# RMichelsen/VulkanHybridRenderer

Hardware: AMD Instinct MI355X
Metric: Mrays/s (unique rays) + ms/frame, Sponza 1080p RT shadows+AO+SVGF (higher is better)
Workload: dtype f32

## Files before the change

include/vhr_amd.h:

```cpp
#ifndef VHR_AMD_H
#define VHR_AMD_H

#include "vhr_types.h"

#ifdef __cplusplus
extern "C" {
#endif

typedef struct vhr_context vhr_context;
typedef struct vhr_raytracing_execution_context vhr_raytracing_execution_context;
typedef struct vhr_compute_execution_context vhr_compute_execution_context;

enum {
    VHR_OK = 0,
    VHR_ERROR_INVALID_ARGUMENT = -1,
    VHR_ERROR_DEVICE = -2,
    VHR_ERROR_NOT_FOUND = -3,
    VHR_ERROR_OUT_OF_SLOTS = -4,
    VHR_ERROR_GRAPH = -5,
    VHR_ERROR_NO_DEVICE = -6,
    VHR_ERROR_UNSUPPORTED = -7
};

enum {
// ... 185 lines not shown
    uint32_t grid_rows, grid_cols;
    uint32_t col_begin, col_end, row_begin, row_end;
    uint32_t overlap;
    uint32_t halo_rows, halo_cols;
    uint32_t col_cut[VHR_TILE_MAX_GRID + 1], row_cut[VHR_TILE_MAX_GRID][VHR_TILE_MAX_GRID + 1];
} vhr_tile_plan;
typedef struct vhr_rect { uint32_t x0, x1, y0, y1; } vhr_rect;
typedef struct vhr_rect_exchange { int32_t peer; vhr_rect send, recv; } vhr_rect_exchange;
#define VHR_COMM_UNIQUE_ID_BYTES 128
typedef struct vhr_comm vhr_comm;

uint32_t vhr_atrous_overlap(uint32_t atrous_steps);
uint32_t vhr_atrous_output_extent(uint32_t overlap, uint32_t step);
int vhr_strip_plan_make(uint32_t height, uint32_t world, uint32_t rank, uint32_t max_motion_rows, uint32_t atrous_steps, vhr_strip_plan *out);
int vhr_strip_plan_exchanges(const vhr_strip_plan *plan, uint32_t n_rows, vhr_row_exchange out[2]);

int vhr_tile_grid_choose(uint32_t width, uint32_t height, uint32_t world, uint32_t overlap, uint32_t *grid_rows, uint32_t *grid_cols);
int vhr_tile_plan_make(uint32_t width, uint32_t height, uint32_t world, uint32_t rank, uint32_t grid_rows, uint32_t grid_cols, uint32_t max_motion_rows,
                       uint32_t max_motion_cols, uint32_t atrous_steps, vhr_tile_plan *out);
int vhr_tile_plan_make_weighted(uint32_t width, uint32_t height, uint32_t world, uint32_t rank, uint32_t grid_rows, uint32_t grid_cols, uint32_t max_motion_rows,
                                uint32_t max_motion_cols, uint32_t atrous_steps, const uint32_t *cost, uint32_t cost_cols, uint32_t cost_rows, uint32_t cell,
                                vhr_tile_plan *out);
int vhr_tile_plan_exchanges(const vhr_tile_plan *plan, uint32_t halo_rows, uint32_t halo_cols, vhr_rect_exchange *out, uint32_t capacity);
int vhr_tile_plan_replan(const vhr_tile_plan *old_plan, const vhr_tile_plan *new_plan, vhr_rect_exchange *out, uint32_t capacity);

int vhr_comm_use_library(const char *path);
const char *vhr_comm_library(void);
int vhr_comm_get_unique_id(uint8_t out[VHR_COMM_UNIQUE_ID_BYTES]);
int vhr_comm_create(vhr_context *ctx, const vhr_strip_plan *plan, const uint8_t unique_id[VHR_COMM_UNIQUE_ID_BYTES], vhr_comm **out);
int vhr_comm_create_tiled(vhr_context *ctx, const vhr_tile_plan *plan, const uint8_t unique_id[VHR_COMM_UNIQUE_ID_BYTES], vhr_comm **out);
void vhr_comm_destroy(vhr_comm *comm);
const char *vhr_comm_last_error(const vhr_comm *comm);
int vhr_comm_exchange_raytraced(vhr_comm *comm, const char *raytraced_image);
int vhr_comm_start_frame_exchanges(vhr_comm *comm, int32_t history_storage_image, int32_t moments_storage_image, const char *denoised_image,
                                   int32_t root, void *gathered_frame);
int vhr_comm_finish_frame_exchanges(vhr_comm *comm);
int vhr_comm_replan(vhr_comm *comm, const vhr_tile_plan *new_plan, int32_t history_storage_image, int32_t moments_storage_image, int32_t prev_normals_storage_image);

int vhr_set_ray_statistics(vhr_context *ctx, int32_t enable);
int vhr_get_ray_statistics(vhr_context *ctx, uint64_t out[4]);

int vhr_set_option(vhr_context *ctx, const char *key, int32_t value);
int vhr_get_option(vhr_context *ctx, const char *key, int32_t *value);
int32_t vhr_option_count(void);
int vhr_option_info(int32_t index, const char **name, int32_t *default_value, int32_t *min_value, int32_t *max_value);

int vhr_set_kernel_timing(vhr_context *ctx, int32_t kind_mask);
int vhr_get_kernel_time(vhr_context *ctx, int32_t kind, double *total_ms, uint64_t *launches, int32_t reset);

const char *vhr_source_fingerprint(void);
int vhr_debug_wave_lifetimes(vhr_context *ctx, uint32_t *out, uint32_t capacity, uint32_t *count);
int vhr_debug_ray_triangle(vhr_context *ctx, const float *pairs, uint32_t count, uint32_t *hit, float *tuv);
int vhr_debug_triangle_records(vhr_context *ctx, int32_t previous, float *out, uint32_t capacity_triangles, uint32_t *count);
int vhr_get_tile_cost_map(vhr_context *ctx, uint32_t *out, uint32_t cols, uint32_t rows);

int vhr_get_traversal_statistics(vhr_context *ctx, uint64_t out[4]);
int vhr_get_reflection_statistics(vhr_context *ctx, uint64_t out[10]);
int vhr_get_binary64_statistics(vhr_context *ctx, uint64_t out[4]);

int vhr_get_traversal_cycles(vhr_context *ctx, uint64_t out[8]);

int vhr_get_drain_statistics(vhr_context *ctx, uint64_t out[4]);

int vhr_calibration_stream_read(vhr_context *ctx, int32_t storage_image, uint32_t bytes_per_lane);

int vhr_get_build_times(vhr_context *ctx, double out[2]);
int vhr_get_bvh_builder(vhr_context *ctx, int32_t *used);
int vhr_get_bvh_presplit_level(vhr_context *ctx, int32_t *level);
int vhr_get_bvh_frame(vhr_context *ctx, float out[9]);

int vhr_get_bvh_statistics(vhr_context *ctx, uint64_t out[5]);
int vhr_get_bvh_form_checks(vhr_context *ctx, uint64_t out[4]);
int vhr_get_bvh_fingerprint(vhr_context *ctx, uint64_t *out);
int vhr_get_bvh_tree_fingerprint(vhr_context *ctx, uint64_t *out);
int vhr_get_bvh_forms_fingerprint(vhr_context *ctx, uint64_t out[2]);

#define VHR_UPDATE_DEVICE_MEMORY 2u
int vhr_update_vertices(vhr_context *ctx, uint32_t first_vertex, uint32_t vertex_count, const vhr_vertex *vertices, uint32_t flags);
int vhr_update_primitive_transforms(vhr_context *ctx, uint32_t first_primitive, uint32_t count, const float *transforms);
int vhr_refit_geometry(vhr_context *ctx);
int vhr_get_refit_statistics(vhr_context *ctx, uint64_t out[8]);
int vhr_get_refit_times(vhr_context *ctx, double out[4]);
#define VHR_REFIT_FORCE_PARTIAL 1u
int vhr_refit_geometry_partial(vhr_context *ctx, uint32_t flags);
int vhr_get_partial_refit_statistics(vhr_context *ctx, uint64_t out[8]);
int vhr_get_object_motion_statistics(vhr_context *ctx, uint64_t out[4]);
int vhr_get_bvh_sah_cost(vhr_context *ctx, double out[2]);

int vhr_ray_query(vhr_context *ctx, const vhr_ray *rays, uint32_t count, uint32_t flags, void *results);
int vhr_ray_query_masked(vhr_context *ctx, const vhr_ray *rays, uint32_t count, uint32_t flags, uint32_t cull_mask, const uint8_t *ray_masks, void *results);
int vhr_get_ray_query_statistics(vhr_context *ctx, uint64_t out[4]);
int vhr_ray_query_struct_layout(uint32_t out[8]);

int vhr_set_primitive_masks(vhr_context *ctx, uint32_t first_primitive, uint32_t count, const uint8_t *masks);
int vhr_get_primitive_masks(vhr_context *ctx, uint32_t first_primitive, uint32_t count, uint8_t *out);
int vhr_get_ray_mask_statistics(vhr_context *ctx, uint64_t out[4]);

#ifdef __cplusplus
}
#endif
#endif
```

vulkanhybridrenderer_amd/csrc/bvh_build.cpp:

```cpp
#include <algorithm>
#include <cmath>
#include <cstring>
#include <cstdlib>
#include <cstdio>
#include <chrono>
#include <atomic>
#include <limits>
#include <queue>
#include <thread>
#include <mutex>
#include <system_error>

#include "vhr_internal.hpp"
#include "presplit.hpp"
#include "bvh_frame.hpp"
#include "bvh_math.hpp"

namespace vhr {
namespace {

struct Box {
    float lo[3], hi[3];
    void reset() {
        for (int a = 0; a < 3; ++a) { lo[a] = std::numeric_limits<float>::infinity(); hi[a] = -std::numeric_limits<float>::infinity(); }
// ... 199 lines not shown
    template <typename F>
    static void run_pool(unsigned threads, size_t n, F &&fn) {
        std::atomic<size_t> next{ 0 };
        auto worker = [&]() { for (size_t k = next.fetch_add(1); k < n; k = next.fetch_add(1)) fn(k); };
        std::vector<std::thread> pool;
        for (unsigned t = 1; t < threads && t < n; ++t) {
            try { pool.emplace_back(worker); } catch (const std::system_error &) { break; }
        }
        worker();
        for (auto &t : pool) t.join();
    }

    void build_parallel(uint32_t n, int threads) {
        const unsigned hw = host_threads(threads);
        if (hw == 1 || n < 32768u) {
            build(nodes, max_depth, 0, n, 0);
            return;
        }
        const uint32_t region = std::max<uint32_t>(16384u, n / 8u), small = std::max<uint32_t>(4096u, n / (8u * hw));
        std::vector<Task> regions;
        top_threads = hw;
        build(nodes, max_depth, 0, n, 0, region, &regions);
        top_threads = 1;
        std::vector<std::vector<TmpNode>> mid(regions.size());
        std::vector<std::vector<Task>> tasks(regions.size());
        std::vector<uint32_t> mid_depth(regions.size(), 0);
        run_pool(hw, regions.size(), [&](size_t k) {
            const Task &r = regions[k];
            build(mid[k], mid_depth[k], r.first, r.count, r.depth, small, r.count > small ? &tasks[k] : nullptr);
        });
        struct Ref { uint32_t region, task; };
        std::vector<Ref> flat;
        for (size_t k = 0; k < regions.size(); ++k)
            for (size_t j = 0; j < tasks[k].size(); ++j) flat.push_back(Ref{ uint32_t(k), uint32_t(j) });
        std::vector<std::vector<std::vector<TmpNode>>> sub(regions.size());
        for (size_t k = 0; k < regions.size(); ++k) sub[k].resize(tasks[k].size());
        std::vector<uint32_t> sub_depth(flat.size(), 0);
        run_pool(hw, flat.size(), [&](size_t f) {
            const Task &t = tasks[flat[f].region][flat[f].task];
            auto &v = sub[flat[f].region][flat[f].task];
            v.reserve(size_t(t.count));
            build(v, sub_depth[f], t.first, t.count, t.depth);
        });
        for (size_t k = 0; k < regions.size(); ++k) splice(mid[k], sub[k]);
        splice(nodes, mid);
        for (uint32_t d : mid_depth) max_depth = std::max(max_depth, d);
        for (uint32_t d : sub_depth) max_depth = std::max(max_depth, d);
    }
};

}

void build_bvh(const vhr_vertex *vertices, const uint32_t *indices, const vhr_primitive *primitives,
               uint32_t primitive_count, HostBvh &out, int leaf_tris, int threads, int presplit_percent, int frame_mode) {
    const bool k0trace = std::getenv("VHR_K0_TRACE") != nullptr; auto k0t = std::chrono::steady_clock::now();
    auto lap = [&](const char *what) { if (k0trace) { auto t = std::chrono::steady_clock::now(); std::fprintf(stderr, "K0 %s %.1f ms\n", what, std::chrono::duration<double, std::milli>(t - k0t).count()); k0t = t; } };
    Builder b;
    b.leaf_tris = std::max(1, std::min(kMaxLeafTris, leaf_tris));
    size_t total = 0;
    for (uint32_t p = 0; p < primitive_count; ++p) total += primitives[p].index_count / 3;
    b.tris.reserve(total);
    for (uint32_t p = 0; p < primitive_count; ++p) {
        const vhr_primitive &pr = primitives[p];
        for (uint32_t t = 0; t < pr.index_count / 3; ++t) {
            const uint32_t *vi = indices + pr.index_offset + 3 * t;
            BvhTri tri;
            bvh_math::world_record(pr.transform, vertices[pr.vertex_offset + vi[0]].pos, vertices[pr.vertex_offset + vi[1]].pos, vertices[pr.vertex_offset + vi[2]].pos, tri.v0,
                                   tri.e1, tri.e2);
            tri.prim = p;
            tri.tri = t;
            tri.flat = uint32_t(b.tris.size());
            b.tris.push_back(tri);
        }
    }
    uint32_t n = uint32_t(b.tris.size());
    out.nodes.clear();
    out.nodes16.clear();
    out.nodes_ch.clear();
    out.nodes48.clear();
    out.tris.clear();
    out.max_depth = 0;
    if (n == 0) return;

    b.tri_box.resize(n);
    b.centroid.resize(size_t(n) * 3);
    b.order.resize(n);
    const unsigned hw = host_threads(threads);
    out.frame_on = false;
    { const float identity[9] = { 1, 0, 0, 0, 1, 0, 0, 0, 1 }; std::memcpy(out.frame, identity, sizeof(identity)); }
    if (frame_mode == 1 && n >= 2u) {
        float frame[9];
        const bool found = bvh_frame::choose([&](const bvh_frame::Candidates &c, uint64_t *sums) {
            for (int k = 0; k < c.n; ++k) sums[k] = 0;
            std::mutex m;
            const size_t stride = bvh_frame::sample_stride(n), samples = (size_t(n) + stride - 1) / stride;
            parallel_for(samples, hw, [&](size_t i0, size_t i1) {
                uint64_t part[bvh_frame::kMaxCandidates] = {};
                for (size_t i = i0; i < i1; ++i)
                    for (int k = 0; k < c.n; ++k) part[k] += bvh_frame::cost_term(c.r[k], b.tris[i * stride]);
                std::lock_guard<std::mutex> lock(m);
                for (int k = 0; k < c.n; ++k) sums[k] += part[k];
            });
        }, frame);
        if (found) { std::memcpy(out.frame, frame, sizeof(frame)); out.frame_on = true; }
        lap("frame search");
    }
    const bool framed = out.frame_on;
// ... 78 lines not shown
        std::vector<int32_t> queue{ 0 };
        for (size_t head = 0; head < queue.size(); ++head) {
            const int32_t id = queue[head];
            int32_t child[4] = { b.nodes[id].left, b.nodes[id].right, -1, -1 };
            int nc = 2;
            while (nc < 4) {
                int best = -1;
                float best_area = -1.0f;
                for (int c = 0; c < nc; ++c) {
                    const TmpNode &t = b.nodes[child[c]];
                    if (t.left < 0) continue;
                    const float area = t.box.half_area();
                    if (area > best_area) { best_area = area; best = c; }
                }
                if (best < 0) break;
                const TmpNode &t = b.nodes[child[best]];
                for (int c = nc; c > best + 1; --c) child[c] = child[c - 1];
                child[best] = t.left;
                child[best + 1] = t.right;
                ++nc;
            }
            for (int c = 0; c < nc; ++c) {
                if (b.nodes[child[c]].left >= 0) queue.push_back(child[c]);
                else { leaf_pos[child[c]] = pos; pos += b.nodes[child[c]].count; }
            }
        }
    }
    out.tris.resize(n);
    parallel_for(b.nodes.size(), hw, [&](size_t i0, size_t i1) {
        for (size_t i = i0; i < i1; ++i) {
            const TmpNode &t = b.nodes[i];
            if (t.left >= 0) continue;
            for (uint32_t j = 0; j < t.count; ++j) out.tris[leaf_pos[i] + j] = b.tris[b.order[t.first + j]];
        }
    });
    lap("triangle order");

    const float inf = std::numeric_limits<float>::infinity();
    auto set_child = [&](BvhNode &node, int which, const TmpNode &child, int32_t link) {
        bvh_math::pad_slot(child.box.lo, child.box.hi, which == 0 ? node.box0 : node.box1);
        (which == 0 ? node.child0 : node.child1) = link;
    };

    const TmpNode &root = b.nodes[0];
    if (root.left < 0) {
        BvhNode node{};
        set_child(node, 0, root, bvh_math::leaf_link(leaf_pos[0], root.count));
        for (int a = 0; a < 3; ++a) { node.box1[2 * a] = inf; node.box1[2 * a + 1] = -inf; }
        node.child1 = node.child0;
        out.nodes.push_back(node);
        derive_node_forms(out, threads);
        return;
    }
    std::vector<int32_t> bfs_index(b.nodes.size(), -1);
    std::vector<int32_t> bfs_order;
    std::queue<int32_t> q;
    q.push(0);
    while (!q.empty()) {
        int32_t id = q.front();
        q.pop();
        bfs_index[id] = int32_t(bfs_order.size());
        bfs_order.push_back(id);
        const TmpNode &t = b.nodes[id];
        if (b.nodes[t.left].left >= 0) q.push(t.left);
        if (b.nodes[t.right].left >= 0) q.push(t.right);
    }
    out.nodes.resize(bfs_order.size());
    parallel_for(bfs_order.size(), hw, [&](size_t k0, size_t k1) {
    for (size_t k = k0; k < k1; ++k) {
        const TmpNode &t = b.nodes[bfs_order[k]];
        BvhNode node{};
        const TmpNode &l = b.nodes[t.left], &r = b.nodes[t.right];
        set_child(node, 0, l, l.left >= 0 ? bfs_index[t.left] : bvh_math::leaf_link(leaf_pos[t.left], l.count));
        set_child(node, 1, r, r.left >= 0 ? bfs_index[t.right] : bvh_math::leaf_link(leaf_pos[t.right], r.count));
        out.nodes[k] = node;
    }
    });
    lap("numbering + (lo, hi) nodes");
    derive_node_forms(out, threads);
    lap("derived node forms");
}

void derive_node_forms(HostBvh &out, int threads, const std::vector<uint8_t> *only) {
    const unsigned hw = host_threads(threads);
    const size_t n = out.nodes.size();
    if (!only) {
        float lo[3], hi[3];
        bvh_math::no_bounds(lo, hi);
        for (const BvhNode &nd : out.nodes) bvh_math::bounds_of_node(nd, lo, hi);
        bvh_math::centre_of(lo, hi, out.centre);
    }
    out.nodes_ch.resize(n);
    out.nodes48.resize(n);
    out.nodes16.resize(n);
    parallel_for(n, hw, [&](size_t k0, size_t k1) {
        for (size_t k = k0; k < k1; ++k)
            if (!only || (*only)[k]) bvh_math::forms_of(out.nodes[k], out.centre, out.nodes_ch[k], out.nodes48[k], out.nodes16[k]);
    });
    out.nodes16_valid = nodes16_in_range(out);
}

namespace {
struct WordHash {
    uint64_t h = 1469598103934665603ull;
    template <typename T>
    void eat(const T *p, size_t count) {
        static_assert(sizeof(T) % 8 == 0, "whole words");
        const unsigned char *b = reinterpret_cast<const unsigned char *>(p);
        for (size_t i = 0; i + 8 <= count * sizeof(T); i += 8) { uint64_t w; std::memcpy(&w, b + i, 8); h = (h ^ w) * 1099511628211ull; h ^= h >> 29; }
    }
};
}
uint64_t bvh_fingerprint(const HostBvh &bvh) {
    WordHash hash;
    hash.eat(bvh.nodes.data(), bvh.nodes.size());
    hash.eat(bvh.tris.data(), bvh.tris.size());
    return hash.h;
}
uint64_t bvh_forms_fingerprint(const HostBvh &bvh) {
    WordHash hash;
    const struct { float c[4]; } centre = { { bvh.centre[0], bvh.centre[1], bvh.centre[2], 0.0f } };
    hash.eat(&centre, 1);
    hash.eat(bvh.nodes_ch.data(), bvh.nodes_ch.size());
    hash.eat(bvh.nodes48.data(), bvh.nodes48.size());
    hash.eat(bvh.nodes16.data(), bvh.nodes16.size());
    return hash.h;
}
// ... 192 lines not shown
```

vulkanhybridrenderer_amd/csrc/bvh_math.hpp:

```cpp
#pragma once

#include <hip/hip_fp16.h>

#include <cmath>
#include <cstdint>
#include <cstring>

#include "vhr_internal.hpp"
#include "bvh_frame.hpp"

namespace vhr {
namespace bvh_math {

#define VHR_BM __host__ __device__ inline

VHR_BM int32_t leaf_link(uint32_t first, uint32_t count) { return ~int32_t((first << 2) | (count - 1u)); }
VHR_BM uint32_t leaf_first(int32_t link) { return ~uint32_t(link) >> 2; }
VHR_BM uint32_t leaf_count(int32_t link) { return (~uint32_t(link) & 3u) + 1u; }
template <typename Node>
VHR_BM int32_t link_as_offset(int32_t link) { return link >= 0 ? link * int32_t(sizeof(Node)) : link; }
VHR_BM bool absent_child1(const BvhNode &nd, bool single) { return single && nd.child1 == nd.child0; }

VHR_BM uint32_t world_record(const float m[16], const float *p0, const float *p1, const float *p2, float v0[3], float e1[3], float e2[3]) {
    const float *p[3] = { p0, p1, p2 };
// ... 210 lines not shown
            }
            if (c - h > lo || c + h < hi) ++bad[1];
            if (c48 != c || hw < h) ++bad[2];
            if (!half_pair_in_range(cb, hb) || !(c16 - h16 <= lo) || !(c16 + h16 >= hi)) ++bad[3];
        }
    }
    if (n48.child0 != link_as_offset<BvhNode48>(nd.child0) || n48.child1 != link_as_offset<BvhNode48>(nd.child1) || ch.child0 != nd.child0 || ch.child1 != nd.child1) ++bad[2];
    if (n16.child0 != link_as_offset<BvhNode16>(nd.child0) || n16.child1 != link_as_offset<BvhNode16>(nd.child1)) ++bad[3];
}

VHR_BM bool inside(const float lo[3], const float hi[3], const float slot[6]) {
    bool in = true;
    for (int a = 0; a < 3; ++a) in = in && lo[a] >= slot[2 * a] && hi[a] <= slot[2 * a + 1];
    return in;
}
VHR_BM void refit_check(const BvhNode &nd, bool single, const BvhNode *nodes, const BvhTri *tris, const float frame[9], bool frame_on, int &records_outside,
                        int &children_outside) {
    for (int which = 0; which < 2; ++which) {
        if (which == 1 && absent_child1(nd, single)) continue;
        const float *slot = which == 0 ? nd.box0 : nd.box1;
        const int32_t link = which == 0 ? nd.child0 : nd.child1;
        if (link >= 0) {
            const BvhNode c = nodes[link];
            for (int w = 0; w < 2; ++w) {
                const float *cb = w == 0 ? c.box0 : c.box1;
                const float lo[3] = { cb[0], cb[2], cb[4] }, hi[3] = { cb[1], cb[3], cb[5] };
                if (!inside(lo, hi, slot)) ++children_outside;
            }
        } else {
            const uint32_t first = leaf_first(link), n = leaf_count(link);
            for (uint32_t i = 0; i < n; ++i) {
                float lo[3], hi[3];
                record_box(tris[first + i], frame, frame_on, lo, hi);
                if (!inside(lo, hi, slot)) ++records_outside;
            }
        }
    }
}

VHR_BM double half_area_of_slot(const float b[6]) {
    const double dx = double(b[1]) - double(b[0]), dy = double(b[3]) - double(b[2]), dz = double(b[5]) - double(b[4]);
    return dx * dy + dy * dz + dz * dx;
}
VHR_BM double sah_term(const float box[6], int32_t link) { return half_area_of_slot(box) * (link >= 0 ? 1.0 : double(leaf_count(link))); }
VHR_BM double sah_cost(double sum, const BvhNode &root, bool single) {
    float box[6];
    for (int i = 0; i < 6; ++i) box[i] = root.box0[i];
    if (!absent_child1(root, single))
        for (int a = 0; a < 3; ++a) { box[2 * a] = fminf(box[2 * a], root.box1[2 * a]); box[2 * a + 1] = fmaxf(box[2 * a + 1], root.box1[2 * a + 1]); }
    const double area = half_area_of_slot(box);
    return area > 0.0 ? sum / area : 0.0;
}

#undef VHR_BM

}
}
```

vulkanhybridrenderer_amd/csrc/context.cpp:

```cpp
#include <cmath>
#include <chrono>
#include <cmath>
#include <cstring>
#include <string>

#include "vhr_internal.hpp"
#include "fingerprint.h"

namespace vhr {
static SrgbLutCopy *g_srgb_lut_copies = nullptr;
SrgbLutCopy::SrgbLutCopy(int (*copy_fn)(const float *)) : copy(copy_fn), next(g_srgb_lut_copies) { g_srgb_lut_copies = this; }
int upload_srgb_lut(const float *lut) {
    if (!g_srgb_lut_copies) return -1;
    for (const SrgbLutCopy *c = g_srgb_lut_copies; c; c = c->next)
        if (c->copy(lut) != 0) return -1;
    return 0;
}

uint32_t format_stride(int32_t format) {
    switch (format) {
        case VHR_FORMAT_R8G8B8A8_UNORM:
        case VHR_FORMAT_R8G8B8A8_SRGB:
        case VHR_FORMAT_B8G8R8A8_UNORM:
        case VHR_FORMAT_B8G8R8A8_SRGB:
// ... 364 lines not shown
    }
    for (uint32_t v = 0; v < vertex_count; ++v)
        if (!std::isfinite(vertices[v].pos[0]) || !std::isfinite(vertices[v].pos[1]) || !std::isfinite(vertices[v].pos[2]))
            return ctx->fail(VHR_ERROR_INVALID_ARGUMENT, "UpdateGeometry: vertex " + std::to_string(v) + " has a non-finite position");
    if (total_triangles >= (1ull << 29))
        return ctx->fail(VHR_ERROR_INVALID_ARGUMENT, "UpdateGeometry: 2^29 triangles or more");
    ctx->scene_can_discard = false;
    for (uint32_t p = 0; p < primitive_count; ++p) {
        const vhr_material &m = primitives[p].material;
        if (m.alpha_mask == 1 || m.base_color_texture != -1 || m.base_color[3] == 0.0f) ctx->scene_can_discard = true;
    }
    ctx->h_prim_masks.clear();
    ctx->mask_present[0] = ctx->mask_present[1] = ctx->mask_present[2] = 0; ctx->mask_present[3] = 1ull << 63;
    ctx->masks_not_ff = 0;
    ctx->refit_pending = ctx->sah_cost_built_valid = false;
    for (uint64_t &w : ctx->refit_stats) w = 0;
    for (uint64_t &w : ctx->partial_stats) w = 0;
    ctx->refit_dirty = RefitDirty{};
    ctx->prim_tri_prefix.assign(size_t(primitive_count) + 1u, 0u);
    for (uint32_t p = 0; p < primitive_count; ++p) ctx->prim_tri_prefix[p + 1u] = ctx->prim_tri_prefix[p] + primitives[p].index_count / 3;
    if (!ctx->host_only) {
        HIP_TRY(ctx, hipSetDevice(ctx->device));
        { const int src_ = ctx->sync_streams(); if (src_ != VHR_OK) return src_; }
        free_scene(ctx);
    }

    auto upload = [&](void **dst, const void *src, size_t bytes) -> hipError_t {
        *dst = nullptr;
        if (bytes == 0) return hipSuccess;
        hipError_t e = hipMalloc(dst, bytes);
        if (e != hipSuccess) return e;
        return hipMemcpy(*dst, src, bytes, hipMemcpyHostToDevice);
    };
    double upload_ms = 0.0;
    if (!ctx->host_only) {
        const auto t0 = std::chrono::steady_clock::now();
        std::vector<float> nm(size_t(primitive_count) * 9);
        for (uint32_t p = 0; p < primitive_count; ++p) normal_matrix3(primitives[p].transform, &nm[size_t(p) * 9]);
        HIP_TRY(ctx, upload(reinterpret_cast<void **>(&ctx->d_vertices), vertices, sizeof(vhr_vertex) * vertex_count));
        HIP_TRY(ctx, upload(reinterpret_cast<void **>(&ctx->d_indices), indices, sizeof(uint32_t) * index_count));
        HIP_TRY(ctx, upload(reinterpret_cast<void **>(&ctx->d_primitives), primitives, sizeof(vhr_primitive) * primitive_count));
        HIP_TRY(ctx, upload(reinterpret_cast<void **>(&ctx->d_normal_matrices), nm.data(), sizeof(float) * nm.size()));
        upload_ms += std::chrono::duration<double, std::milli>(std::chrono::steady_clock::now() - t0).count();
    }

    HostBvh bvh;
    bool device_built = false;
    ctx->bvh_builder_used = 0;
    if (ctx->bvh_builder >= 1 && !ctx->host_only && total_triangles >= 2ull * uint64_t(ctx->bvh_leaf_tris)) {
        std::vector<uint32_t> prefix(primitive_count);
        uint32_t acc = 0;
        for (uint32_t p = 0; p < primitive_count; ++p) { prefix[p] = acc; acc += primitives[p].index_count / 3; }
        const auto t0 = std::chrono::steady_clock::now();
        const int rc = device_build_bvh(ctx, prefix, uint32_t(total_triangles), ctx->bvh_leaf_tris, ctx->bvh_presplit, ctx->bvh_frame_mode);
        const auto t1 = std::chrono::steady_clock::now();
        if (rc == VHR_OK) {
            device_built = true;
            ctx->bvh_builder_used = 1;
            ctx->bvh_build_ms = std::chrono::duration<double, std::milli>(t1 - t0).count();
            ctx->bvh_fingerprint_valid = false;
            if (ctx->bvh_host_checks) {
                const int frc = fetch_device_tree(ctx, bvh);
                if (frc != VHR_OK) return frc;
            }
        } else {
            hipFree(ctx->d_nodes); hipFree(ctx->d_nodes16); hipFree(ctx->d_nodes_ch); hipFree(ctx->d_nodes48); hipFree(ctx->d_tris);
            ctx->d_nodes = nullptr; ctx->d_nodes16 = nullptr; ctx->d_nodes_ch = nullptr; ctx->d_nodes48 = nullptr; ctx->d_tris = nullptr;
            ctx->node_count = ctx->tri_count = 0;
            if (rc != VHR_ERROR_OUT_OF_SLOTS) return rc;
        }
    }
    const auto t_build0 = std::chrono::steady_clock::now();
    if (!device_built) {
        build_bvh(vertices, indices, primitives, primitive_count, bvh, ctx->bvh_leaf_tris, ctx->bvh_build_threads, ctx->bvh_presplit, ctx->bvh_frame_mode);
        ctx->bvh_build_ms = std::chrono::duration<double, std::milli>(std::chrono::steady_clock::now() - t_build0).count();
        ctx->bvh_presplit_level = bvh.presplit_level;
        for (int i = 0; i < 9; ++i) ctx->bvh_frame[i] = bvh.frame[i];
        ctx->bvh_frame_on = bvh.frame_on;
    }
    if (uint64_t(device_built ? ctx->node_count : bvh.nodes48.size()) * sizeof(BvhNode48) >= (1ull << 31))
        return ctx->fail(VHR_ERROR_INVALID_ARGUMENT, "UpdateGeometry: more than 44 million BVH nodes");
    const auto t_build1 = std::chrono::steady_clock::now();
    if (!device_built || ctx->bvh_host_checks) {
        check_node_forms(bvh, ctx->bvh_form_checks, ctx->bvh_build_threads);
        ctx->nodes16_valid = bvh.nodes16_valid && ctx->bvh_form_checks[3] == 0;
        ctx->bvh_fingerprint = bvh_fingerprint(bvh);
        ctx->bvh_tree_fingerprint = bvh_tree_fingerprint(bvh);
        ctx->bvh_fingerprint_valid = true;
    }
    ctx->bvh_check_ms = std::chrono::duration<double, std::milli>(std::chrono::steady_clock::now() - t_build1).count();
    if (ctx->host_only) {
        ctx->node_count = uint32_t(bvh.nodes.size());
        ctx->tri_count = uint32_t(bvh.tris.size());
        ctx->bvh_depth = bvh.max_depth;
        ctx->geometry_upload_ms = 0.0;
        ctx->h_vertices.assign(vertices, vertices + vertex_count);
        ctx->h_indices.assign(indices, indices + index_count);
        ctx->h_primitives.assign(primitives, primitives + primitive_count);
        ctx->h_bvh = std::move(bvh);
        ctx->vertex_count = vertex_count;
        ctx->index_count = index_count;
        ctx->primitive_count = primitive_count;
        return reset_motion(ctx);
    }
    if (!device_built) {
        const auto t_upload0 = std::chrono::steady_clock::now();
        HIP_TRY(ctx, upload(reinterpret_cast<void **>(&ctx->d_nodes), bvh.nodes.data(), sizeof(BvhNode) * bvh.nodes.size()));
        HIP_TRY(ctx, upload(reinterpret_cast<void **>(&ctx->d_nodes16), bvh.nodes16.data(), sizeof(BvhNode16) * bvh.nodes16.size()));
        HIP_TRY(ctx, upload(reinterpret_cast<void **>(&ctx->d_nodes_ch), bvh.nodes_ch.data(), sizeof(BvhNodeCH) * bvh.nodes_ch.size()));
        HIP_TRY(ctx, upload(reinterpret_cast<void **>(&ctx->d_nodes48), bvh.nodes48.data(), sizeof(BvhNode48) * bvh.nodes48.size()));
        HIP_TRY(ctx, upload(reinterpret_cast<void **>(&ctx->d_tris), bvh.tris.data(), sizeof(BvhTri) * bvh.tris.size()));
        for (int a = 0; a < 3; ++a) ctx->bvh_centre[a] = bvh.centre[a];
        ctx->node_count = uint32_t(bvh.nodes.size());
        ctx->tri_count = uint32_t(bvh.tris.size());
        ctx->bvh_depth = bvh.max_depth;
        upload_ms += std::chrono::duration<double, std::milli>(std::chrono::steady_clock::now() - t_upload0).count();
    }
    ctx->vertex_count = vertex_count;
    ctx->index_count = index_count;
    ctx->primitive_count = primitive_count;
    ctx->geometry_upload_ms = upload_ms;
    return reset_motion(ctx);
}

int vhr_get_bvh_builder(vhr_context *ctx, int32_t *used) {
    if (!ctx || !used) return VHR_ERROR_INVALID_ARGUMENT;
    *used = ctx->bvh_builder_used;
// ... 362 lines not shown
    if (!ctx || !p) return VHR_ERROR_INVALID_ARGUMENT;
    if (p->ao_spp > 64) return ctx->fail(VHR_ERROR_INVALID_ARGUMENT, "trace params: ao_spp > 64");
    ctx->trace_params = *p;
    return VHR_OK;
}

int vhr_set_tile(vhr_context *ctx, uint32_t col_begin, uint32_t col_end, uint32_t row_begin, uint32_t row_end, uint32_t overlap,
                 uint32_t halo_rows, uint32_t halo_cols) {
    if (!ctx || row_begin > row_end || row_end > ctx->height || col_begin > col_end || col_end > ctx->width || halo_rows < overlap || halo_cols < overlap)
        return ctx ? ctx->fail(VHR_ERROR_INVALID_ARGUMENT, "set_tile: need begin <= end <= extent on both axes and halos >= overlap") : VHR_ERROR_INVALID_ARGUMENT;
    ctx->row_begin = row_begin;
    ctx->row_end = row_end;
    ctx->col_begin = col_begin;
    ctx->col_end = col_end;
    ctx->overlap = overlap;
    ctx->halo = halo_rows;
    ctx->halo_cols = halo_cols;
    return VHR_OK;
}

int vhr_set_strip(vhr_context *ctx, uint32_t row_begin, uint32_t row_end, uint32_t overlap, uint32_t halo) {
    if (!ctx || row_begin > row_end || row_end > ctx->height || halo < overlap)
        return ctx ? ctx->fail(VHR_ERROR_INVALID_ARGUMENT, "set_strip: need row_begin <= row_end <= height and halo >= overlap") : VHR_ERROR_INVALID_ARGUMENT;
    return vhr_set_tile(ctx, 0, ctx->width, row_begin, row_end, overlap, halo, std::max(halo, ctx->width));
}

int vhr_set_option(vhr_context *ctx, const char *key, int32_t value) {
    if (!ctx || !key) return VHR_ERROR_INVALID_ARGUMENT;
    if (!std::strcmp(key, "bvh_leaf_triangles")) {
        if (value < 1 || value > kMaxLeafTris) return ctx->fail(VHR_ERROR_INVALID_ARGUMENT, "bvh_leaf_triangles must be 1..4");
        ctx->bvh_leaf_tris = value;
        return VHR_OK;
    }
    if (!std::strcmp(key, "bvh_host_checks")) {
        if (value < 0 || value > 1) return ctx->fail(VHR_ERROR_INVALID_ARGUMENT, "bvh_host_checks must be 0 or 1");
        ctx->bvh_host_checks = value;
        return VHR_OK;
    }
    if (!std::strcmp(key, "bvh_device_max_depth")) {
        if (value < 1 || value > kMaxBvhDepth) return ctx->fail(VHR_ERROR_INVALID_ARGUMENT, "bvh_device_max_depth must be 1..40");
        ctx->bvh_device_max_depth = value;
        return VHR_OK;
    }
    if (!std::strcmp(key, "bvh_builder")) {
        if (value < 0 || value > 1) return ctx->fail(VHR_ERROR_INVALID_ARGUMENT, "bvh_builder must be 0 (binned SAH on the host) or 1 (binned SAH on the device)");
        ctx->bvh_builder = value;
        return VHR_OK;
    }
    if (!std::strcmp(key, "bvh_frame")) {
        if (value < 0 || value > 1) return ctx->fail(VHR_ERROR_INVALID_ARGUMENT, "bvh_frame must be 0 (boxes along the world axes) or 1 (along the frame that minimises the triangles' summed box area)");
        ctx->bvh_frame_mode = value;
        return VHR_OK;
    }
    if (!std::strcmp(key, "bvh_presplit")) {
        if (value < 0 || value > 400) return ctx->fail(VHR_ERROR_INVALID_ARGUMENT, "bvh_presplit must be 0 (off) or the budget of extra triangle references in percent (1..400)");
        ctx->bvh_presplit = value;
        return VHR_OK;
    }
    if (!std::strcmp(key, "bvh_build_threads")) {
        if (value < 0 || value > 64) return ctx->fail(VHR_ERROR_INVALID_ARGUMENT, "bvh_build_threads must be 0..64");
        ctx->bvh_build_threads = value;
        return VHR_OK;
    }
    if (!std::strcmp(key, "alpha_test_rays")) {
        if (value < 0 || value > 1) return ctx->fail(VHR_ERROR_INVALID_ARGUMENT, "alpha_test_rays must be 0 (every triangle is opaque to the hybrid path's rays) or 1 (they skip what the G-buffer pass discards)");
        ctx->alpha_test_rays = value;
        return VHR_OK;
    }
    {
        int *const slot = !std::strcmp(key, "shadow_ray_mask") ? &ctx->shadow_ray_mask : !std::strcmp(key, "ao_ray_mask") ? &ctx->ao_ray_mask :
                          !std::strcmp(key, "reflection_ray_mask") ? &ctx->reflection_ray_mask : nullptr;
        if (slot) {
            if (value < 0 || value > 255) return ctx->fail(VHR_ERROR_INVALID_ARGUMENT, std::string(key) + " must be 0..255 (a primitive whose mask shares no bit with it does not exist for that class of rays)");
            *slot = value;
            return VHR_OK;
        }
    }
    if (!std::strcmp(key, "object_motion_vectors")) {
        if (value < 0 || value > 1)
            return ctx->fail(VHR_ERROR_INVALID_ARGUMENT, "object_motion_vectors must be 0 (motion vectors follow the camera only) or 1 (and the geometry the refits moved)");
        if (ctx->recording || ctx->cur_pass) return ctx->fail(VHR_ERROR_GRAPH, "object_motion_vectors: set from inside a pass");
        if (value == ctx->object_motion_vectors) return VHR_OK;
        if (!ctx->host_only) {
            HIP_TRY(ctx, hipSetDevice(ctx->device));
            const int src_ = ctx->sync_streams(); if (src_ != VHR_OK) return src_;
        }
        ctx->object_motion_vectors = value;
        const int rc = reset_motion(ctx);
        if (rc != VHR_OK) ctx->object_motion_vectors = 0;
        return rc;
    }
    for (int i = 0; i < vhr::kOptCount; ++i) {
        const vhr::OptionInfo &o = vhr::kOptionInfo[i];
        if (std::strcmp(key, o.name)) continue;
        if (value < o.lo || value > o.hi)
            return ctx->fail(VHR_ERROR_INVALID_ARGUMENT, std::string(o.name) + " must be " + std::to_string(o.lo) + ".." + std::to_string(o.hi));
        ctx->options[i] = value;
        return VHR_OK;
    }
    return ctx->fail(VHR_ERROR_NOT_FOUND, std::string("unknown option '") + key + "'");
}

int32_t vhr_option_count(void) { return vhr::kOptCount; }

int vhr_option_info(int32_t index, const char **name, int32_t *default_value, int32_t *min_value, int32_t *max_value) {
    if (index < 0 || index >= vhr::kOptCount) return VHR_ERROR_INVALID_ARGUMENT;
    const vhr::OptionInfo &o = vhr::kOptionInfo[index];
    if (name) *name = o.name;
    if (default_value) *default_value = o.def;
    if (min_value) *min_value = o.lo;
    if (max_value) *max_value = o.hi;
    return VHR_OK;
}

int vhr_get_option(vhr_context *ctx, const char *key, int32_t *value) {
    if (!ctx || !key || !value) return VHR_ERROR_INVALID_ARGUMENT;
    if (!std::strcmp(key, "alpha_test_rays")) { *value = ctx->alpha_test_rays; return VHR_OK; }
    if (!std::strcmp(key, "object_motion_vectors")) { *value = ctx->object_motion_vectors; return VHR_OK; }
    if (!std::strcmp(key, "shadow_ray_mask")) { *value = ctx->shadow_ray_mask; return VHR_OK; }
    if (!std::strcmp(key, "ao_ray_mask")) { *value = ctx->ao_ray_mask; return VHR_OK; }
    if (!std::strcmp(key, "reflection_ray_mask")) { *value = ctx->reflection_ray_mask; return VHR_OK; }
    for (int i = 0; i < vhr::kOptCount; ++i)
        if (!std::strcmp(key, vhr::kOptionInfo[i].name)) { *value = ctx->options[i]; return VHR_OK; }
    return ctx->fail(VHR_ERROR_NOT_FOUND, std::string("unknown option '") + key + "'");
}

int vhr_set_ray_statistics(vhr_context *ctx, int32_t enable) {
    if (!ctx) return VHR_ERROR_INVALID_ARGUMENT;
    ctx->ray_stats_enabled = enable != 0;
    return VHR_OK;
}

int vhr_get_ray_statistics(vhr_context *ctx, uint64_t out[4]) {
    if (!ctx || !out) return VHR_ERROR_INVALID_ARGUMENT;
    if (!ctx->host_only) { const int src_ = ctx->sync_streams(); if (src_ != VHR_OK) return src_; }
    const vhr_trace_params &tp = ctx->trace_params;
    const uint64_t covered = ctx->h_ray_stats.covered_pixels;
    if (ctx->raytraced_pixels) {
        out[0] = out[1] = ctx->raytraced_pixels + covered;
        out[2] = covered;
        out[3] = ctx->h_ray_stats.stack_overflows;
        return VHR_OK;
    }
    const uint64_t second = ctx->h_ray_stats.second_bounce_rays;
    out[0] = covered * (uint64_t(tp.shadow_enable ? 1 : 0) + tp.ao_spp + (tp.reflections ? 1 : 0)) + second;
    out[1] = covered * (uint64_t(tp.shadow_enable ? 4 : 0) + tp.ao_spp + (tp.reflections ? 1 : 0)) + second;
    out[2] = covered;
    out[3] = ctx->h_ray_stats.stack_overflows;
    return VHR_OK;
}

int vhr_get_traversal_statistics(vhr_context *ctx, uint64_t out[4]) {
    if (!ctx || !out) return VHR_ERROR_INVALID_ARGUMENT;
    if (!ctx->host_only) { const int src_ = ctx->sync_streams(); if (src_ != VHR_OK) return src_; }
    out[0] = ctx->h_ray_stats.node_visits; out[1] = ctx->h_ray_stats.leaf_visits;
    out[2] = ctx->h_ray_stats.triangle_tests; out[3] = ctx->h_ray_stats.wave_iterations;
    return VHR_OK;
}

int vhr_get_reflection_statistics(vhr_context *ctx, uint64_t out[10]) {
    if (!ctx || !out) return VHR_ERROR_INVALID_ARGUMENT;
    if (!ctx->host_only) { const int src_ = ctx->sync_streams(); if (src_ != VHR_OK) return src_; }
    const RayStats &r = ctx->h_refl_stats;
    out[0] = r.unique_rays; out[1] = r.second_bounce_rays; out[2] = r.node_visits; out[3] = r.leaf_visits; out[4] = r.triangle_tests;
    out[5] = r.wave_iterations; out[6] = r.refills; out[7] = r.waves; out[8] = r.cycles_total; out[9] = r.cycles_nodes;
    return VHR_OK;
}

int vhr_get_binary64_statistics(vhr_context *ctx, uint64_t out[4]) {
    if (!ctx || !out) return VHR_ERROR_INVALID_ARGUMENT;
// ... 78 lines not shown
    return VHR_OK;
}

int vhr_ray_query_struct_layout(uint32_t out[8]) {
    if (!out) return VHR_ERROR_INVALID_ARGUMENT;
    out[0] = sizeof(vhr_ray); out[1] = offsetof(vhr_ray, tmin); out[2] = offsetof(vhr_ray, direction); out[3] = offsetof(vhr_ray, tmax);
    out[4] = sizeof(vhr_ray_hit); out[5] = offsetof(vhr_ray_hit, geometry_index); out[6] = offsetof(vhr_ray_hit, primitive_index);
    out[7] = offsetof(vhr_ray_hit, reserved);
    return 8;
}

int vhr_calibration_stream_read(vhr_context *ctx, int32_t storage_image, uint32_t bytes_per_lane) {
    if (!ctx || ctx->host_only || storage_image < 0 || uint32_t(storage_image) >= vhr_context::kMaxGlobalResources || !ctx->storage_images[storage_image].used)
        return ctx ? ctx->fail(VHR_ERROR_NOT_FOUND, "calibration: no such storage image") : VHR_ERROR_INVALID_ARGUMENT;
    return launch_calibration_read(ctx, ctx->storage_images[storage_image], bytes_per_lane, ctx->d_tile_counter);
}

int vhr_debug_ray_triangle(vhr_context *ctx, const float *pairs, uint32_t count, uint32_t *hit, float *tuv) {
    if (!ctx || (count && (!pairs || !hit || !tuv))) return ctx ? ctx->fail(VHR_ERROR_INVALID_ARGUMENT, "vhr_debug_ray_triangle: null argument") : VHR_ERROR_INVALID_ARGUMENT;
    if (ctx->host_only) return ctx->fail(VHR_ERROR_DEVICE, "vhr_debug_ray_triangle: host-only context");
    return launch_ray_triangle_pairs(ctx, pairs, count, hit, tuv);
}

int vhr_debug_triangle_records(vhr_context *ctx, int32_t previous, float *out, uint32_t capacity_triangles, uint32_t *count) {
    if (!ctx || !count || (previous != 0 && previous != 1)) return ctx ? ctx->fail(VHR_ERROR_INVALID_ARGUMENT, "vhr_debug_triangle_records: null count, or previous is neither 0 nor 1") : VHR_ERROR_INVALID_ARGUMENT;
    *count = 0;
    if (ctx->host_only ? ctx->h_bvh.nodes.empty() : (ctx->d_nodes == nullptr || ctx->node_count == 0))
        return ctx->fail(VHR_ERROR_GRAPH, "vhr_debug_triangle_records: no geometry yet (vhr_update_geometry first)");
    if (ctx->bvh_presplit_level >= 0)
        return ctx->fail(VHR_ERROR_UNSUPPORTED, "vhr_debug_triangle_records: the tree was built with \"bvh_presplit\" and has several records per triangle: there is no record per flat triangle to report");
    if (previous && !ctx->motion_valid())
        return ctx->fail(VHR_ERROR_GRAPH, "vhr_debug_triangle_records: no previous records (vhr_set_option \"object_motion_vectors\" 1 first)");
    *count = ctx->tri_count;
    if (capacity_triangles < ctx->tri_count || !out)
        return ctx->fail(VHR_ERROR_INVALID_ARGUMENT, "vhr_debug_triangle_records: room for " + std::to_string(capacity_triangles) + " triangles, the scene has " + std::to_string(ctx->tri_count));
    std::vector<BvhTri> fetched;
    const BvhTri *records = previous ? ctx->h_bvh.prev_tris.data() : ctx->h_bvh.tris.data();
    if (!ctx->host_only) {
        HIP_TRY(ctx, hipSetDevice(ctx->device));
        { const int src_ = ctx->sync_streams(); if (src_ != VHR_OK) return src_; }
        fetched.resize(ctx->tri_count);
        HIP_TRY(ctx, hipMemcpy(fetched.data(), previous ? ctx->d_prev_tris : ctx->d_tris, sizeof(BvhTri) * ctx->tri_count, hipMemcpyDeviceToHost));
        records = fetched.data();
    }
    for (uint32_t k = 0; k < ctx->tri_count; ++k) {
        const BvhTri &t = records[k];
        if (t.flat >= ctx->tri_count) return ctx->fail(VHR_ERROR_GRAPH, "vhr_debug_triangle_records: a record's flat index lies outside the scene's triangles");
        float *o = out + size_t(t.flat) * 9;
        for (int c = 0; c < 3; ++c) { o[c] = t.v0[c]; o[3 + c] = t.e1[c]; o[6 + c] = t.e2[c]; }
    }
    return VHR_OK;
}

int vhr_get_object_motion_statistics(vhr_context *ctx, uint64_t out[4]) {
    if (!ctx || !out) return VHR_ERROR_INVALID_ARGUMENT;
    out[0] = ctx->motion_valid() ? 1u : 0u;
    out[1] = ctx->motion_valid() ? ctx->motion_differing : 0u;
    out[2] = ctx->motion_launches;
    out[3] = 0;
    return VHR_OK;
}

int vhr_get_bvh_statistics(vhr_context *ctx, uint64_t out[5]) {
    if (!ctx || !out) return VHR_ERROR_INVALID_ARGUMENT;
    out[0] = ctx->node_count; out[1] = ctx->tri_count; out[2] = ctx->bvh_depth;
    out[3] = uint64_t(ctx->node_count) * sizeof(BvhNode); out[4] = uint64_t(ctx->tri_count) * sizeof(BvhTri);
    return VHR_OK;
}

const char *vhr_source_fingerprint(void) { return VHR_SOURCE_FINGERPRINT; }

int vhr_debug_wave_lifetimes(vhr_context *ctx, uint32_t *out, uint32_t capacity, uint32_t *count) {
    if (!ctx || !out || !count) return VHR_ERROR_INVALID_ARGUMENT;
    const int src_ = ctx->sync_streams(); if (src_ != VHR_OK) return src_;
    const vhr_context::CostOrder &co = ctx->cost_order_raygen;
    const uint32_t n = std::min<uint32_t>(capacity, co.cost_blocks[co.slot] ? std::min(co.cost_waves[co.slot], co.capacity) : 0u);
    *count = n;
    if (n && hipMemcpy(out, co.cost[co.slot], size_t(n) * 4, hipMemcpyDeviceToHost) != hipSuccess) return ctx->fail(VHR_ERROR_DEVICE, "wave lifetimes: copy failed");
    return VHR_OK;
}

int vhr_get_tile_cost_map(vhr_context *ctx, uint32_t *out, uint32_t cols, uint32_t rows) {
    if (!ctx || !out || cols == 0 || rows == 0) return VHR_ERROR_INVALID_ARGUMENT;
    if (ctx->host_only) return ctx->fail(VHR_ERROR_NO_DEVICE, "host-only context: no device work");
    if (uint64_t(cols) * 8 < ctx->width || uint64_t(rows) * 8 < ctx->height) return ctx->fail(VHR_ERROR_INVALID_ARGUMENT, "tile cost map: the map does not cover the image");
    const int src_ = ctx->sync_streams(); if (src_ != VHR_OK) return src_;
    std::fill(out, out + size_t(cols) * rows, 0u);
    std::vector<uint32_t> host;
    int found = 0;
    for (const vhr_context::CostOrder *co : { &ctx->cost_order_raygen, &ctx->cost_order_reflection }) {
        const uint32_t slot = co->slot;
        const vhr_context::CostOrder::Shape &sh = co->shape[slot];
        const uint32_t n = co->cost_blocks[slot] ? std::min(co->cost_waves[slot], co->capacity) : 0u;
        if (!n || !sh.tiles_x) continue;
        host.resize(n);
        if (hipMemcpy(host.data(), co->cost[slot], size_t(n) * 4, hipMemcpyDeviceToHost) != hipSuccess) return ctx->fail(VHR_ERROR_DEVICE, "tile cost map: copy failed");
        for (uint32_t i = 0; i < n; ++i) {
            const uint32_t block = i / sh.wv, wave = i % sh.wv;
            const uint32_t by = block / sh.blocks_x, bx = block % sh.blocks_x;
            const uint32_t x = sh.col_begin + (bx * sh.wv + wave) * sh.tile_w, y = sh.row_begin + by * sh.tile_h;
            if (x >= ctx->width || y >= ctx->height) continue;
            uint32_t &cell = out[size_t(y / 8) * cols + x / 8];
            cell = uint32_t(std::min<uint64_t>(0xffffffffull, uint64_t(cell) + host[i]));
        }
        ++found;
    }
// ... 263 lines not shown
```

vulkanhybridrenderer_amd/csrc/kernels_bvh.hip:

```cpp
#include <hipcub/hipcub.hpp>

#include <algorithm>
#include <cmath>
#include <cstdio>
#include <cstdlib>
#include <cstring>
#include <chrono>
#include <vector>

#include "vhr_internal.hpp"
#include "presplit.hpp"
#include "bvh_frame.hpp"
#include "bvh_math.hpp"

namespace vhr {
namespace {

struct Box6 { float lo[3], hi[3]; };

__device__ __forceinline__ uint32_t ordered(float f) {
    const uint32_t u = __float_as_uint(f);
    return (u & 0x80000000u) ? ~u : (u | 0x80000000u);
}
__host__ __device__ inline float unordered(uint32_t u) {
// ... 19 lines not shown
        uint32_t lo = 0, hi = primitive_count;
        while (hi - lo > 1u) { const uint32_t mid = (lo + hi) >> 1; if (tri_prefix[mid] <= t) lo = mid; else hi = mid; }
        const uint32_t p = lo, local = t - tri_prefix[p];
        const vhr_primitive &pr = primitives[p];
        const uint32_t *vi = indices + pr.index_offset + 3u * local;
        BvhTri tri;
        Box6 b;
        bvh_math::world_record(pr.transform, vertices[pr.vertex_offset + vi[0]].pos, vertices[pr.vertex_offset + vi[1]].pos, vertices[pr.vertex_offset + vi[2]].pos, tri.v0, tri.e1,
                               tri.e2);
        bvh_math::record_box(tri, nullptr, false, b.lo, b.hi);
#pragma unroll
        for (int a = 0; a < 3; ++a) c[a] = 0.5f * (b.lo[a] + b.hi[a]);
        tri.prim = p;
        tri.tri = local;
        tri.flat = t;
        tris[t] = tri;
        boxes[t] = b;
    }
#pragma unroll
    for (int a = 0; a < 3; ++a) {
        float mn = t < n ? c[a] : 3.0e38f, mx = t < n ? c[a] : -3.0e38f;
        for (int off = 32; off > 0; off >>= 1) { mn = fminf(mn, __shfl_xor(mn, off)); mx = fmaxf(mx, __shfl_xor(mx, off)); }
        if ((threadIdx.x & 63u) == 0u) { atomic_min_checked(&centre_bounds[a], ordered(mn)); atomic_max_checked(&centre_bounds[3 + a], ordered(mx)); }
    }
}

__global__ __launch_bounds__(256) void k0_positions_kernel(const int2 *__restrict__ node_children, const uint32_t *__restrict__ node_parent,
                                                           const uint32_t *__restrict__ node_size, uint32_t n, uint32_t root, uint32_t leaf_tris,
                                                           uint32_t *__restrict__ position, uint32_t *__restrict__ max_depth) {
    const uint32_t k = blockIdx.x * 256u + threadIdx.x;
    if (k >= n) return;
    uint32_t pos = 0, depth = 0, node = k;
    while (node != root) {
        const uint32_t parent = node_parent[node];
        const int2 ch = node_children[parent];
        if (uint32_t(ch.y) == node) pos += node_size[uint32_t(ch.x)];
        if (node_size[parent] > leaf_tris) ++depth;
        node = parent;
    }
    position[k] = pos;
    atomicMax(max_depth, depth);
}
__global__ __launch_bounds__(256) void k0_place_triangles_kernel(const BvhTri *__restrict__ tris_flat, const uint32_t *__restrict__ sorted_vals,
                                                                 const uint32_t *__restrict__ position, uint32_t n, BvhTri *__restrict__ tris_out) {
    const uint32_t k = blockIdx.x * 256u + threadIdx.x;
    if (k < n) tris_out[position[k]] = tris_flat[sorted_vals[k]];
}
__device__ __forceinline__ uint32_t first_triangle(const int2 *node_children, const uint32_t *position, uint32_t n, uint32_t node) {
    while (node >= n) node = uint32_t(node_children[node].x);
    return position[node];
}
__global__ __launch_bounds__(256) void k0_emit_kernel(const int2 *__restrict__ node_children, const Box6 *__restrict__ node_box, const uint32_t *__restrict__ node_size,
                                                      const uint32_t *__restrict__ kept_rank, const uint32_t *__restrict__ position, uint32_t n, uint32_t total_nodes,
                                                      uint32_t leaf_tris, BvhNode *__restrict__ nodes) {
    const uint32_t node = n + blockIdx.x * 256u + threadIdx.x;
    if (node >= total_nodes || node_size[node] <= leaf_tris) return;
    const int2 ch = node_children[node];
    auto link_of = [&](uint32_t c) -> int32_t {
        const uint32_t size = node_size[c];
        if (size > leaf_tris) return int32_t(kept_rank[c - n]);
        return bvh_math::leaf_link(first_triangle(node_children, position, n, c), size);
    };
    BvhNode out{};
    const Box6 b0 = node_box[uint32_t(ch.x)], b1 = node_box[uint32_t(ch.y)];
    bvh_math::pad_slot(b0.lo, b0.hi, out.box0);
    bvh_math::pad_slot(b1.lo, b1.hi, out.box1);
    out.child0 = link_of(uint32_t(ch.x));
    out.child1 = link_of(uint32_t(ch.y));
    nodes[kept_rank[node - n]] = out;
}
__global__ __launch_bounds__(256) void k0_kept_flags_kernel(const uint32_t *__restrict__ node_size, uint32_t n, uint32_t total_nodes, uint32_t leaf_tris, uint32_t *__restrict__ flags) {
    const uint32_t k = blockIdx.x * 256u + threadIdx.x;
    if (n + k < total_nodes) flags[k] = node_size[n + k] > leaf_tris ? 1u : 0u;
}

__device__ __forceinline__ bool node_selected(const uint32_t *dirty, uint32_t k) { return !dirty || ((dirty[k >> 5] >> (k & 31u)) & 1u) != 0u; }
__global__ __launch_bounds__(256) void k0_forms_kernel(const BvhNode *__restrict__ nodes, uint32_t count, float cx, float cy, float cz, BvhNodeCH *__restrict__ nodes_ch,
                                                       BvhNode48 *__restrict__ nodes48, BvhNode16 *__restrict__ nodes16, const uint32_t *__restrict__ dirty) {
    const uint32_t k = blockIdx.x * 256u + threadIdx.x;
    if (k >= count || !node_selected(dirty, k)) return;
    const BvhNode nd = nodes[k];
    const float centre[3] = { cx, cy, cz };
    BvhNodeCH c;
    BvhNode48 n48;
    BvhNode16 h16;
    bvh_math::forms_of(nd, centre, c, n48, h16);
    nodes_ch[k] = c;
    nodes16[k] = h16;
    nodes48[k] = n48;
}

__global__ __launch_bounds__(256) void k0_check_forms_kernel(const BvhNode *__restrict__ nodes, const BvhNodeCH *__restrict__ nodes_ch, const BvhNode48 *__restrict__ nodes48,
                                                             const BvhNode16 *__restrict__ nodes16, uint32_t count, float cx, float cy, float cz,
                                                             unsigned long long *__restrict__ out, const uint32_t *__restrict__ dirty, uint16_t *__restrict__ status) {
    const uint32_t k = blockIdx.x * 256u + threadIdx.x;
    uint32_t bad[5] = { 0u, 0u, 0u, 0u, 0u };
    uint32_t old = 0u;
    if (k < count && node_selected(dirty, k)) {
        const BvhNode nd = nodes[k];
        const BvhNodeCH ch = nodes_ch[k];
        const BvhNode48 n48 = nodes48[k];
        const BvhNode16 n16 = nodes16[k];
        const float centre[3] = { cx, cy, cz };
        bvh_math::check_forms(nd, ch, n48, n16, centre, bad);
        if (status) {
            if (dirty) old = status[k];
            status[k] = uint16_t(bad[1] | (bad[2] << 4) | (bad[3] << 8) | (bad[4] << 12));
        }
    }
#pragma unroll
    for (int i = 0; i < 5; ++i) {
        int v = int(bad[i]) - (i ? int((old >> (4 * (i - 1))) & 15u) : 0);
        for (int off = 32; off > 0; off >>= 1) v += __shfl_xor(v, off);
        if ((threadIdx.x & 63u) == 0u && v) atomicAdd(&out[i], (unsigned long long)(long long)v);
    }
}

__global__ __launch_bounds__(256) void k0_node_bounds_kernel(const BvhNode *__restrict__ nodes, uint32_t count, uint32_t *__restrict__ bounds) {
    const uint32_t k = blockIdx.x * 256u + threadIdx.x;
    float mn[3], mx[3];
    bvh_math::no_bounds(mn, mx);
// ... 661 lines not shown
        const uint32_t old = dirty ? status[k] : 0u;
        status[k] = uint8_t(uint32_t(bad_records) | (uint32_t(bad_children) << 4));
        bad_records -= int(old & 15u);
        bad_children -= int(old >> 4);
    }
    for (int off = 32; off > 0; off >>= 1) { bad_records += __shfl_xor(bad_records, off); bad_children += __shfl_xor(bad_children, off); }
    if ((threadIdx.x & 63u) == 0u) {
        if (bad_records) atomicAdd(&counters->records_outside, (unsigned long long)(long long)bad_records);
        if (bad_children) atomicAdd(&counters->children_outside, (unsigned long long)(long long)bad_children);
    }
}
__global__ __launch_bounds__(256) void k0_sah_cost_kernel(const BvhNode *__restrict__ nodes, uint32_t count, double *__restrict__ partial) {
    __shared__ double s_wave[4];
    const uint32_t k = blockIdx.x * 256u + threadIdx.x;
    double sum = 0.0;
    if (k < count) {
        const BvhNode nd = nodes[k];
        sum = bvh_math::sah_term(nd.box0, nd.child0);
        if (!bvh_math::absent_child1(nd, count == 1u)) sum += bvh_math::sah_term(nd.box1, nd.child1);
    }
    for (int off = 32; off > 0; off >>= 1) sum += __shfl_xor(sum, off);
    if ((threadIdx.x & 63u) == 0u) s_wave[threadIdx.x >> 6] = sum;
    __syncthreads();
    if (threadIdx.x == 0u) partial[blockIdx.x] = ((s_wave[0] + s_wave[1]) + s_wave[2]) + s_wave[3];
}

void centre_from_bounds(const uint32_t bounds[6], float centre[3]) {
    float lo[3], hi[3];
    for (int a = 0; a < 3; ++a) { lo[a] = unordered(bounds[a]); hi[a] = unordered(bounds[3 + a]); }
    bvh_math::centre_of(lo, hi, centre);
}

struct Scratch {
    std::vector<void *> ptrs;
    template <typename T>
    hipError_t alloc(T **p, size_t count) {
        *p = nullptr;
        if (!count) return hipSuccess;
        const hipError_t e = hipMalloc(reinterpret_cast<void **>(p), count * sizeof(T));
        if (e == hipSuccess) ptrs.push_back(*p);
        return e;
    }
    ~Scratch() { for (void *p : ptrs) hipFree(p); }
};

}

#define K0_TRY(expr)                                                                                       \
    do {                                                                                                    \
        hipError_t e_ = (expr);                                                                             \
        if (e_ != hipSuccess) return ctx->fail(VHR_ERROR_DEVICE, std::string("device K0: ") + #expr + ": " + hipGetErrorString(e_)); \
    } while (0)

int device_build_bvh(vhr_context *ctx, const std::vector<uint32_t> &tri_prefix, uint32_t total_tris, int leaf_tris_in, int presplit_percent, int frame_mode) {
    uint32_t n = total_tris;
    const uint32_t leaf_tris = uint32_t(std::max(1, std::min(kMaxLeafTris, leaf_tris_in)));
    if (n <= leaf_tris || n < 2u) return VHR_ERROR_OUT_OF_SLOTS;
    hipStream_t s = ctx->stream;
    Scratch tmp;
    const bool trace = std::getenv("VHR_K0_TRACE") != nullptr;
    auto t_last = std::chrono::steady_clock::now();
    auto lap = [&](const char *what) {
        if (!trace) return;
        (void)hipStreamSynchronize(s);
        const auto now = std::chrono::steady_clock::now();
        std::fprintf(stderr, "K0 device %s %.2f ms\n", what, std::chrono::duration<double, std::milli>(now - t_last).count());
        t_last = now;
    };
    const dim3 block(256);
    auto grid = [](uint32_t count) { return dim3((count + 255u) / 256u); };
    uint32_t *d_prefix, *d_bounds, *d_counts;
    BvhTri *d_tris_flat;
    Box6 *d_boxes;
    K0_TRY(tmp.alloc(&d_prefix, tri_prefix.size()));
    K0_TRY(tmp.alloc(&d_bounds, 12));
    K0_TRY(tmp.alloc(&d_counts, 4));
    K0_TRY(tmp.alloc(&d_tris_flat, n)); K0_TRY(tmp.alloc(&d_boxes, n));
    K0_TRY(hipMemcpyAsync(d_prefix, tri_prefix.data(), tri_prefix.size() * sizeof(uint32_t), hipMemcpyHostToDevice, s));
    const uint32_t init_bounds[12] = { 0xffffffffu, 0xffffffffu, 0xffffffffu, 0u, 0u, 0u, 0xffffffffu, 0xffffffffu, 0xffffffffu, 0u, 0u, 0u };
    K0_TRY(hipMemcpyAsync(d_bounds, init_bounds, sizeof(init_bounds), hipMemcpyHostToDevice, s));
    K0_TRY(hipMemsetAsync(d_counts, 0, 4 * sizeof(uint32_t), s));
    hipLaunchKernelGGL(k0_triangles_kernel, grid(n), block, 0, s, ctx->d_vertices, ctx->d_indices, ctx->d_primitives, d_prefix, uint32_t(tri_prefix.size()), n,
                       d_tris_flat, d_boxes, d_bounds);
    uint32_t h_bounds[12];
    K0_TRY(hipMemcpyAsync(h_bounds, d_bounds, sizeof(h_bounds), hipMemcpyDeviceToHost, s));
    K0_TRY(hipStreamSynchronize(s));
    ctx->bvh_frame_on = false;
    { const float identity[9] = { 1, 0, 0, 0, 1, 0, 0, 0, 1 }; std::memcpy(ctx->bvh_frame, identity, sizeof(identity)); }
    if (frame_mode == 1) {
        unsigned long long *d_sums;
        K0_TRY(tmp.alloc(&d_sums, size_t(bvh_frame::kMaxCandidates)));
        hipError_t pass_error = hipSuccess;
        float frame[9];
        const uint32_t stride = bvh_frame::sample_stride(n), samples = (n + stride - 1u) / stride;
        const bool found = bvh_frame::choose([&](const bvh_frame::Candidates &c, uint64_t *sums) {
            static_assert(sizeof(uint64_t) == sizeof(unsigned long long), "64-bit sums");
            hipError_t e = hipMemsetAsync(d_sums, 0, sizeof(unsigned long long) * bvh_frame::kMaxCandidates, s);
            if (e == hipSuccess) { hipLaunchKernelGGL(k0_frame_cost_kernel, grid(samples), block, 0, s, d_tris_flat, samples, stride, c, d_sums); e = hipGetLastError(); }
            if (e == hipSuccess) e = hipMemcpyAsync(sums, d_sums, sizeof(uint64_t) * size_t(c.n), hipMemcpyDeviceToHost, s);
            if (e == hipSuccess) e = hipStreamSynchronize(s);
            if (e != hipSuccess) { pass_error = e; for (int k = 0; k < c.n; ++k) sums[k] = ~0ull; }
        }, frame);
        K0_TRY(pass_error);
        if (found) {
            FrameMatrix fm;
            std::memcpy(fm.r, frame, sizeof(frame));
            K0_TRY(hipMemcpyAsync(d_bounds, init_bounds, sizeof(init_bounds), hipMemcpyHostToDevice, s));
// ... 115 lines not shown
        hipLaunchKernelGGL(k0_sah_flags_kernel, grid(n), block, 0, s, d_boxes, d_order[cur], d_pos_node[cur], d_active[cur], d_splits, n, d_flags);
        K0_TRY(hipcub::DeviceScan::ExclusiveSum(d_work, scan_bytes, d_flags, d_scan, int(n), s));
        hipLaunchKernelGGL(k0_sah_scatter_kernel, grid(n), block, 0, s, d_boxes, d_order[cur], d_pos_node[cur], d_active[cur], d_splits, d_flags, d_scan, n, d_order[cur ^ 1],
                           d_pos_node[cur ^ 1], d_node_box, d_active[cur ^ 1]);
        hipLaunchKernelGGL(k0_sah_fix_boxes_kernel, grid(n_active), block, 0, s, d_splits, n_active, d_node_box);
        K0_TRY(hipMemcpyAsync(&h_counters, d_counters, sizeof(h_counters), hipMemcpyDeviceToHost, s));
        K0_TRY(hipStreamSynchronize(s));
        if (h_counters.error) return VHR_ERROR_OUT_OF_SLOTS;
        if (h_counters.next_active > max_active || h_counters.small_roots > max_small) return ctx->fail(VHR_ERROR_DEVICE, "device K0: a node list overflowed");
        if (trace) std::fprintf(stderr, "K0 device level %d: %u nodes -> %u, %u small roots\n", level, n_active, h_counters.next_active, h_counters.small_roots);
        n_active = h_counters.next_active;
        n_small = h_counters.small_roots;
        cur ^= 1;
    }
    if (n_active) return VHR_ERROR_OUT_OF_SLOTS;
    lap("levels");
    if (n_small) hipLaunchKernelGGL(k0_sah_small_kernel, dim3((n_small + 3u) / 4u), block, 0, s, d_boxes, d_order[cur], d_small, n_small, n, d_counters, d_children, d_parent,
                                    d_size, d_node_box, d_place, depth_guard, leaf_tris);
    hipLaunchKernelGGL(k0_sah_leaves_kernel, grid(n), block, 0, s, d_boxes, d_order[cur], n, d_node_box, d_size);
    K0_TRY(hipMemcpyAsync(&h_counters, d_counters, sizeof(h_counters), hipMemcpyDeviceToHost, s));
    K0_TRY(hipStreamSynchronize(s));
    K0_TRY(hipGetLastError());
    if (h_counters.error) return VHR_ERROR_OUT_OF_SLOTS;
    lap("small subtrees");
    if (h_counters.inner != n - 1u) return ctx->fail(VHR_ERROR_DEVICE, "device K0: the splits did not end in one binary tree");
    const uint32_t total_nodes = 2u * n - 1u, root_id = n;
    uint32_t h_size_root = n;
    K0_TRY(hipMemcpyAsync(d_size + root_id, &h_size_root, 4, hipMemcpyHostToDevice, s));
    hipLaunchKernelGGL(k0_positions_kernel, grid(n), block, 0, s, d_children, d_parent, d_size, n, root_id, leaf_tris, d_position, d_counts);
    hipLaunchKernelGGL(k0_place_triangles_kernel, grid(n), block, 0, s, d_tris_flat, d_order[cur], d_position, n, ctx->d_tris);
    const uint32_t n_inner_all = total_nodes - n;
    hipLaunchKernelGGL(k0_kept_flags_kernel, grid(n_inner_all), block, 0, s, d_size, n, total_nodes, leaf_tris, d_kept);
    K0_TRY(hipcub::DeviceScan::ExclusiveSum(d_work, scan_bytes, d_kept, d_kept_rank, int(n_inner_all), s));
    uint32_t last_rank = 0, last_flag = 0, h_depth = 0;
    K0_TRY(hipMemcpyAsync(&last_rank, d_kept_rank + n_inner_all - 1, 4, hipMemcpyDeviceToHost, s));
    K0_TRY(hipMemcpyAsync(&last_flag, d_kept + n_inner_all - 1, 4, hipMemcpyDeviceToHost, s));
    K0_TRY(hipMemcpyAsync(&h_depth, d_counts, 4, hipMemcpyDeviceToHost, s));
    K0_TRY(hipStreamSynchronize(s));
    const uint32_t n_inner = last_rank + last_flag;
    if (n_inner == 0) return VHR_ERROR_OUT_OF_SLOTS;
    K0_TRY(hipMalloc(reinterpret_cast<void **>(&ctx->d_nodes), sizeof(BvhNode) * n_inner));
    K0_TRY(hipMalloc(reinterpret_cast<void **>(&ctx->d_nodes_ch), sizeof(BvhNodeCH) * n_inner));
    K0_TRY(hipMalloc(reinterpret_cast<void **>(&ctx->d_nodes48), sizeof(BvhNode48) * n_inner));
    K0_TRY(hipMalloc(reinterpret_cast<void **>(&ctx->d_nodes16), sizeof(BvhNode16) * n_inner));
    {
        size_t sort_bytes = 0;
        K0_TRY(hipcub::DeviceRadixSort::SortPairs(nullptr, sort_bytes, d_keys[0], d_keys[1], d_vals[0], d_vals[1], int(n_inner_all), 0, 40, s));
        char *d_sort_work;
        K0_TRY(tmp.alloc(&d_sort_work, sort_bytes));
        hipLaunchKernelGGL(k0_bfs_keys_kernel, grid(n_inner_all), block, 0, s, d_size, d_place, n, total_nodes, leaf_tris, d_keys[0], d_vals[0]);
        K0_TRY(hipcub::DeviceRadixSort::SortPairs(d_sort_work, sort_bytes, d_keys[0], d_keys[1], d_vals[0], d_vals[1], int(n_inner_all), 0, 40, s));
        hipLaunchKernelGGL(k0_bfs_rank_kernel, grid(n_inner), block, 0, s, d_vals[1], n_inner, d_kept_rank);
    }
    hipLaunchKernelGGL(k0_emit_kernel, grid(n_inner_all), block, 0, s, d_children, d_node_box, d_size, d_kept_rank, d_position, n, total_nodes, leaf_tris, ctx->d_nodes);
    hipLaunchKernelGGL(k0_node_bounds_kernel, grid(n_inner), block, 0, s, ctx->d_nodes, n_inner, d_bounds + 6);
    K0_TRY(hipMemcpyAsync(h_bounds, d_bounds, sizeof(h_bounds), hipMemcpyDeviceToHost, s));
    K0_TRY(hipStreamSynchronize(s));
    K0_TRY(hipGetLastError());
    centre_from_bounds(h_bounds + 6, ctx->bvh_centre);
    hipLaunchKernelGGL(k0_forms_kernel, grid(n_inner), block, 0, s, ctx->d_nodes, n_inner, ctx->bvh_centre[0], ctx->bvh_centre[1], ctx->bvh_centre[2], ctx->d_nodes_ch,
                       ctx->d_nodes48, ctx->d_nodes16, static_cast<const uint32_t *>(nullptr));
    {
        unsigned long long *d_checks;
        K0_TRY(tmp.alloc(&d_checks, 5));
        K0_TRY(hipMemsetAsync(d_checks, 0, 5 * sizeof(unsigned long long), s));
        hipLaunchKernelGGL(k0_check_forms_kernel, grid(n_inner), block, 0, s, ctx->d_nodes, ctx->d_nodes_ch, ctx->d_nodes48, ctx->d_nodes16, n_inner,
                           ctx->bvh_centre[0], ctx->bvh_centre[1], ctx->bvh_centre[2], d_checks, static_cast<const uint32_t *>(nullptr), static_cast<uint16_t *>(nullptr));
        unsigned long long h_checks[5];
        K0_TRY(hipMemcpyAsync(h_checks, d_checks, sizeof(h_checks), hipMemcpyDeviceToHost, s));
        K0_TRY(hipStreamSynchronize(s));
        const bool in_range = h_checks[4] == 0ull && size_t(n_inner) * sizeof(BvhNode16) < (size_t(1) << 31);
        for (int i = 0; i < 3; ++i) ctx->bvh_form_checks[i] = h_checks[i];
        ctx->bvh_form_checks[3] = in_range ? h_checks[3] : 0ull;
        ctx->nodes16_valid = in_range && h_checks[3] == 0ull;
    }
    K0_TRY(hipStreamSynchronize(s));
    K0_TRY(hipGetLastError());
    lap("layout + node forms + self-checks");
    ctx->node_count = n_inner;
    ctx->tri_count = n;
    ctx->bvh_depth = h_depth;
    if (std::getenv("VHR_K0_TRACE")) std::fprintf(stderr, "K0 device: %u triangles, %u inner nodes, depth %u\n", n, n_inner, h_depth);
    if (h_depth > uint32_t(std::min(kMaxBvhDepth, ctx->bvh_device_max_depth))) return VHR_ERROR_OUT_OF_SLOTS;
    return VHR_OK;
}

struct RefitPlan {
    std::vector<uint32_t> level_begin;
    Box6 *d_self_box = nullptr;
    RefitCounters *d_counters = nullptr;
    double *d_partial = nullptr;
    uint32_t *d_parent = nullptr;
    uint32_t *d_owner = nullptr;
    uint32_t *d_dirty = nullptr;
    uint16_t *d_form_status = nullptr;
    uint8_t *d_check_status = nullptr;
    bool boxes_valid = false;
    bool dirty_stale = false;
    unsigned long long totals[6] = { 0, 0, 0, 0, 0, 0 };
    hipEvent_t ev[5] = { nullptr, nullptr, nullptr, nullptr, nullptr };
    uint32_t launches = 0;
};
void free_refit_plan(vhr_context *ctx) {
    RefitPlan *p = ctx->refit_plan;
    if (!p) return;
    hipFree(p->d_self_box); hipFree(p->d_counters); hipFree(p->d_partial);
    hipFree(p->d_parent); hipFree(p->d_owner); hipFree(p->d_dirty); hipFree(p->d_form_status); hipFree(p->d_check_status);
// ... 276 lines not shown
```

vulkanhybridrenderer_amd/csrc/kernels_ray_query.hip:

```cpp
#define VHR_TRACE_UNIT unit_ray_query
#include "trace_queue.hpp"

namespace vhr {

__global__ __launch_bounds__(256) void ray_triangle_pairs_kernel(const float *pairs, const uint32_t n, uint32_t *hit, float *tuv, const Stamps st) {
    vhr_stamp(st);
    const uint32_t i = blockIdx.x * 256u + threadIdx.x;
    if (i >= n) return;
    const float *p = pairs + size_t(i) * 17u;
    float t = 0.0f, u = 0.0f, v = 0.0f;
    const bool h = ray_triangle(f3{ p[0], p[1], p[2] }, f3{ p[3], p[4], p[5] }, f3{ p[6], p[7], p[8] }, f3{ p[9], p[10], p[11] }, f3{ p[12], p[13], p[14] }, p[15], p[16], t, u, v);
    hit[i] = h ? 1u : 0u;
    tuv[size_t(i) * 3u] = h ? t : 0.0f; tuv[size_t(i) * 3u + 1u] = h ? u : 0.0f; tuv[size_t(i) * 3u + 2u] = h ? v : 0.0f;
}

int launch_ray_triangle_pairs(vhr_context *ctx, const float *pairs, uint32_t n, uint32_t *hit, float *tuv) {
    if (n == 0) return VHR_OK;
    float *d_pairs = nullptr, *d_tuv = nullptr;
    uint32_t *d_hit = nullptr;
    const size_t pb = size_t(n) * 17u * sizeof(float), tb = size_t(n) * 3u * sizeof(float), hb = size_t(n) * sizeof(uint32_t);
    int rc = VHR_OK;
    if (hipMalloc(&d_pairs, pb) != hipSuccess || hipMalloc(&d_tuv, tb) != hipSuccess || hipMalloc(&d_hit, hb) != hipSuccess)
        rc = ctx->fail(VHR_ERROR_DEVICE, "vhr_debug_ray_triangle: device allocation failed");
    if (rc == VHR_OK && hipMemcpyAsync(d_pairs, pairs, pb, hipMemcpyHostToDevice, ctx->stream) != hipSuccess) rc = ctx->fail(VHR_ERROR_DEVICE, "vhr_debug_ray_triangle: upload failed");
    if (rc == VHR_OK) {
        launch(ctx, ray_triangle_pairs_kernel, dim3((n + 255u) / 256u), dim3(256), 0, static_cast<const float *>(d_pairs), n, d_hit, d_tuv);
        if (hipGetLastError() != hipSuccess || hipMemcpyAsync(hit, d_hit, hb, hipMemcpyDeviceToHost, ctx->stream) != hipSuccess ||
            hipMemcpyAsync(tuv, d_tuv, tb, hipMemcpyDeviceToHost, ctx->stream) != hipSuccess || hipStreamSynchronize(ctx->stream) != hipSuccess)
            rc = ctx->fail(VHR_ERROR_DEVICE, "vhr_debug_ray_triangle: launch or download failed");
    }
    (void)hipFree(d_pairs); (void)hipFree(d_tuv); (void)hipFree(d_hit);
    return rc;
}

#ifndef VHR_QUERY_WAVE_RAYS
#define VHR_QUERY_WAVE_RAYS 256
#endif
constexpr uint32_t kQueryWaveRays = VHR_QUERY_WAVE_RAYS;

struct RayQueryArgs {
    DeviceScene scene;
    const float4 *rays;
    void *results;
    uint32_t *redo_list;
    RayQueryCounters *counters;
    uint32_t count, any_hit;
    RayMaskArgs masks;
    const uint8_t *ray_masks;
};
static_assert(sizeof(vhr_ray) == 2 * sizeof(float4), "vhr_ray is two float4");

__device__ __forceinline__ void ray_query_store(const RayQueryArgs &a, const uint32_t ray, const bool any_hit, const bool hit, const float t,
                                                const float u, const float v, const uint32_t prim, const uint32_t tri) {
    if (any_hit) { static_cast<uint8_t *>(a.results)[ray] = hit ? 1u : 0u; return; }
    uint32_t *const r = static_cast<uint32_t *>(a.results) + size_t(ray) * 6u;
    r[0] = hit ? __float_as_uint(t) : 0u; r[1] = hit ? __float_as_uint(u) : 0u; r[2] = hit ? __float_as_uint(v) : 0u;
    r[3] = hit ? prim : kNoHit; r[4] = hit ? tri : kNoHit; r[5] = 0u;
}

template <bool SPILL, int FILTER = kFilterNone>
__global__ __launch_bounds__(kQueueBlock * 2) void ray_query_kernel(const RayQueryArgs a, const uint32_t stack_levels, const uint32_t refill_threshold,
                                                                    const uint32_t early_exit, const Stamps st) {
    vhr_stamp(st);
    extern __shared__ int s_dyn[];
    const uint32_t lane = threadIdx.x & 63u, wave = uint32_t(__builtin_amdgcn_readfirstlane(int(threadIdx.x >> 6)));
    const uint64_t first = (uint64_t(blockIdx.x) * 2u + wave) * kQueryWaveRays;
    if (first >= a.count) return;
    const uint32_t base = uint32_t(first), total = uint32_t(min(uint64_t(kQueryWaveRays), uint64_t(a.count) - first));
    const bool any_hit = a.any_hit != 0u;
    if (a.scene.node_count == 0) {
        for (uint32_t r = lane; r < total; r += 64u) ray_query_store(a, base + r, any_hit, false, 0.0f, 0.0f, 0.0f, 0u, 0u);
        return;
    }
    int *stack = s_dyn + wave * (stack_levels + 3u) * kQueueBlock + lane;
    stack[0] = kStackSentinel;
    uint32_t overflow = 0, hits = 0;
    bool flagged = false;
    wave_queue_walk<SPILL, false, true, false, true>(
        a.scene, stack, stack_levels, lane, total, refill_threshold, early_exit, 0.0f, 0.0f, any_hit, overflow, nullptr, 0u,
        [&](uint32_t r, uint32_t &ray, f3 &ro, f3 &rd, float &tmin, float &tmax) {
            ray = base + r;
            const float4 p = a.rays[size_t(ray) * 2u], q = a.rays[size_t(ray) * 2u + 1u];
            ro = f3{ p.x, p.y, p.z }; tmin = p.w;
            rd = f3{ q.x, q.y, q.z }; tmax = q.w;
        },
        [&](uint32_t ray, uint32_t tri, float u, float v, float t) {
            const bool hit = tri != kNoHit;
            hits += hit ? 1u : 0u;
            ray_query_store(a, ray, any_hit, hit, t, u, v, hit ? a.scene.tris[tri].prim : 0u, hit ? a.scene.tris[tri].tri : 0u);
            if (flagged) {
                a.redo_list[atomicAdd(&a.counters->redo_count, 1u)] = ray;
                flagged = false;
            }
        }, nullptr,
        [&](uint32_t) { flagged = true; }, ray_filter<FILTER>(a.scene, a.masks, a.masks.shadow, a.ray_masks));
    for (int off = 32; off > 0; off >>= 1) hits += uint32_t(__shfl_xor(int(hits), off));
    const bool wave_overflow = __any(overflow != 0u);
    if (lane == 0) {
        if (hits) atomicAdd(&a.counters->hits, (unsigned long long)hits);
        if (wave_overflow) atomicAdd(&a.counters->overflows, 1u);
    }
}

template <int FILTER = kFilterNone>
__global__ __launch_bounds__(kTraceBlock) void ray_query_redo_kernel(const RayQueryArgs a, const Stamps st) {
    vhr_stamp(st);
    __shared__ int s_stack[kTraceStack * kTraceBlock];
    const uint32_t n = a.counters->redo_count;
    const bool any_hit = a.any_hit != 0u;
    uint32_t overflow = 0;
    int delta = 0;
    for (uint32_t i = blockIdx.x * kTraceBlock + threadIdx.x; i < n; i += gridDim.x * kTraceBlock) {
        const uint32_t ray = a.redo_list[i];
        const float4 p = a.rays[size_t(ray) * 2u], q = a.rays[size_t(ray) * 2u + 1u];
        const f3 o = f3{ p.x, p.y, p.z }, d = f3{ q.x, q.y, q.z };
        Hit best;
        best.t = best.u = best.v = 0.0f; best.tri_index = 0; best.flat = 0;
        bool hit, was;
        uint32_t ray_mask = a.masks.shadow;
        if constexpr (FILTER == kFilterMask) { if (a.ray_masks) ray_mask &= uint32_t(a.ray_masks[ray]); }
        if (any_hit) {
            was = static_cast<const uint8_t *>(a.results)[ray] != 0u;
            hit = traverse<true>(a.scene, o, d, p.w, q.w, s_stack + threadIdx.x, best, overflow, ray_filter<FILTER>(a.scene, a.masks, ray_mask));
        } else {
            was = static_cast<const uint32_t *>(a.results)[size_t(ray) * 6u + 3u] != kNoHit;
            hit = traverse<false>(a.scene, o, d, p.w, q.w, s_stack + threadIdx.x, best, overflow, ray_filter<FILTER>(a.scene, a.masks, ray_mask));
        }
        ray_query_store(a, ray, any_hit, hit, best.t, best.u, best.v, hit && !any_hit ? a.scene.tris[best.tri_index].prim : 0u,
                        hit && !any_hit ? a.scene.tris[best.tri_index].tri : 0u);
        delta += int(hit) - int(was);
    }
    if (delta) atomicAdd(&a.counters->hits, (unsigned long long)(long long)delta);
    if (overflow) atomicAdd(&a.counters->overflows, 1u);
}

int launch_ray_query(vhr_context *ctx, const vhr_ray *rays, uint32_t count, bool any_hit, bool alpha_test, void *results, uint32_t cull_mask,
                     const uint8_t *ray_masks) {
    ctx->rq_mask_ran = 0;
    if (count == 0) return VHR_OK;
    RayQueryScratch *q = nullptr;
    for (RayQueryScratch &e : ctx->rq_scratch) if (e.stream == ctx->stream) q = &e;
    if (!q) {
        ctx->rq_scratch.push_back(RayQueryScratch{ ctx->stream, nullptr, nullptr, 0 });
        q = &ctx->rq_scratch.back();
        if (hipMalloc(reinterpret_cast<void **>(&q->counters), sizeof(RayQueryCounters)) != hipSuccess) {
            q->counters = nullptr;
            ctx->rq_scratch.pop_back();
            return ctx->fail(VHR_ERROR_DEVICE, "vhr_ray_query: device allocation failed");
        }
    }
    if (q->capacity < count) {
        (void)hipFree(q->list);
        q->list = nullptr;
        q->capacity = 0;
        if (hipMalloc(reinterpret_cast<void **>(&q->list), size_t(count) * sizeof(uint32_t)) != hipSuccess)
            return ctx->fail(VHR_ERROR_DEVICE, "vhr_ray_query: device allocation failed");
        q->capacity = count;
    }
    ctx->rq_last_counters = q->counters;
    RayQueryArgs a;
    a.scene = ctx->device_scene();
    a.rays = reinterpret_cast<const float4 *>(rays);
    a.results = results;
    a.redo_list = q->list;
    a.counters = q->counters;
    a.count = count;
    a.any_hit = any_hit ? 1u : 0u;
    if (hipMemsetAsync(q->counters, 0, sizeof(RayQueryCounters), ctx->stream) != hipSuccess)
        return ctx->fail(VHR_ERROR_DEVICE, "vhr_ray_query: hipMemsetAsync failed");
    const QueueLaunch ql = queue_launch(ctx, kOptLdsStackLevels, kOptEarlyExit, 2u);
    const dim3 grid(uint32_t((uint64_t(count) + 2u * kQueryWaveRays - 1u) / (2u * kQueryWaveRays)));
    const bool alpha = alpha_test && ctx->scene_can_discard;
    const bool mask_acts = ray_masks != nullptr || ctx->ray_mask_acts(cull_mask);
    a.masks = RayMaskArgs{ nullptr, cull_mask, cull_mask, cull_mask, alpha ? 1u : 0u };
    a.ray_masks = ray_masks;
    if (mask_acts) {
        if (const int rc = ensure_device_prim_masks(ctx)) return rc;
        a.masks.prim_masks = ctx->d_prim_masks;
        ctx->rq_mask_ran = 1;
    }
    const int filter = launch_filter(mask_acts, alpha);
    ctx->time_begin(kKernelRayQuery);
    with_bool(ql.spill, [&](auto sp) { with_filter(filter, [&](auto al) {
        launch(ctx, ray_query_kernel<decltype(sp)::value, decltype(al)::value>, grid, dim3(kQueueBlock * 2), ql.lds_bytes, a, ql.levels, ql.threshold, ql.early_exit);
    }); });
    if (a.scene.node_count != 0) {
        const uint32_t redo_blocks = std::min<uint32_t>((count + kTraceBlock - 1u) / kTraceBlock, uint32_t(ctx->cu_count) * 4u);
        with_filter(filter, [&](auto al) { launch(ctx, ray_query_redo_kernel<decltype(al)::value>, dim3(redo_blocks), dim3(kTraceBlock), 0, a); });
    }
    ctx->time_end(kKernelRayQuery);
    if (hipGetLastError() != hipSuccess) return ctx->fail(VHR_ERROR_DEVICE, "vhr_ray_query: kernel launch failed");
    return VHR_OK;
}

}
```

vulkanhybridrenderer_amd/csrc/kernels_trace.hip:

```cpp
#define VHR_TRACE_UNIT unit_trace
#include <cstring>

#include "trace_queue.hpp"
#include "svgf_temporal.hpp"

namespace vhr {

#ifndef VHR_REDO_INLINE
#define VHR_REDO_INLINE __attribute__((noinline))
#endif
#ifndef VHR_K1_WAVES_MIN
#define VHR_K1_WAVES_MIN 8
#endif
constexpr uint32_t kRedoPixel = 0x80000000u;

struct RaygenArgs {
    DeviceScene scene;
    vhr_per_frame_data pfd;
    vhr_trace_params tp;
    const void *normals;
    const float *depth;
    void *shadow_ao;
    void *reflections;
    uint32_t width, height;
// ... 50 lines not shown
    float shadow_payload, ao_payload;
    pixel_visibility<1, FILTER>(*a, x, y, a->depth[size_t(y) * a->width + x], st, overflow, P, N, origin, shadow_payload, ao_payload);
    return float2{ shadow_payload, ao_payload };
}

template <int FILTER = kFilterNone>
__device__ __forceinline__ void raygen_pixel(const RaygenArgs &a, const uint32_t x, const uint32_t y, int *stack, uint32_t &overflow, bool &covered, bool &second_ray) {
    const uint32_t W = a.width;
    const float depth = a.depth[size_t(y) * W + x];
    if (depth == 0.0f) {
        store_rg16f(a.shadow_ao, W, x, y, 1.0f, 1.0f);
        if (a.reflections) store_rgba16f(a.reflections, W, x, y, 0.0f, 0.0f, 0.0f, 0.0f);
        return;
    }
    covered = true;
    f3 P, N, origin;
    float shadow_payload, ao_payload;
    pixel_visibility<kTraceBlock, FILTER>(a, x, y, depth, stack, overflow, P, N, origin, shadow_payload, ao_payload);
    store_rg16f(a.shadow_ao, W, x, y, shadow_payload, ao_payload);

    if (a.reflections) {
        f4 payload = f4{ 0.0f, 0.0f, 0.0f, 0.0f };
        if (a.tp.reflections) {
            const f3 cam = f3{ a.pfd.camera_view_inverse[12], a.pfd.camera_view_inverse[13], a.pfd.camera_view_inverse[14] };
            const f3 I = normalize3(P - cam);
            const float ni2 = 2.0f * dot3(N, I);
            const f3 rdir = I - N * ni2;
            payload = trace_reflection<kTraceBlock>(a.scene, a.pfd, a.tp, origin, rdir, stack, overflow, second_ray, ray_filter<FILTER>(a.scene, a.masks, a.masks.reflection));
        }
        store_rgba16f(a.reflections, W, x, y, payload.x, payload.y, payload.z, payload.w);
    }
}

template <int FILTER = kFilterNone>
__global__ __launch_bounds__(kTraceBlock) void raygen_kernel(const RaygenArgs a, const Stamps st) {
    vhr_stamp(st);
    __shared__ int s_stack[kTraceStack * kTraceBlock];
    int *stack = s_stack + threadIdx.x;
    uint32_t x, y;
    pixel_of_thread(x, y, a.row_begin);
    uint32_t overflow = 0;
    bool covered = false, second_ray = false;
    if (x < a.width && y < a.row_end) raygen_pixel<FILTER>(a, x, y, stack, overflow, covered, second_ray);
    if (a.stats) {
        const unsigned long long cov = __ballot(covered), ovf = __ballot(overflow != 0), sec = __ballot(second_ray);
        if ((threadIdx.x & 63u) == 0) {
            if (cov) atomicAdd(&a.stats->covered_pixels, (unsigned long long)__popcll(cov));
            if (ovf) atomicAdd(&a.stats->stack_overflows, (unsigned long long)__popcll(ovf));
            if (sec) atomicAdd(&a.stats->second_bounce_rays, (unsigned long long)__popcll(sec));
        }
    }
}

template <int WAVES, bool COMPACT, bool SPILL, bool STATS, bool FUSE = false, int FILTER = kFilterNone>
__global__ __launch_bounds__(kQueueBlock *WAVES) __attribute__((amdgpu_waves_per_eu(VHR_K1_WAVES_MIN, 8))) void raygen_queue_kernel(const RaygenArgs a, const uint32_t stack_levels, const uint32_t refill_threshold,
                                                                          const uint32_t block_tiles_x, const uint32_t early_exit, const uint32_t tile_rows, const uint32_t steal_threshold, const Stamps st) {
    vhr_stamp(st);
    RayStats *const stats = STATS ? a.stats : nullptr;
    extern __shared__ int s_dyn[];
    const unsigned long long t_start = stats ? __builtin_readcyclecounter() : 0ull;
    unsigned long long t_setup = 0, t_refill = 0, t_nodes = 0, t_leaves = 0, n_refills = 0;
    __shared__ uint32_t s_vis_all[WAVES][kQueueBlock];
    __shared__ float s_ray_all[WAVES][5][kQueueBlock];
    __shared__ uint8_t s_list_all[WAVES][kQueueBlock];
    __shared__ float4 s_cut_all[WAVES][kCutMax][2];
    const uint32_t lane = threadIdx.x & 63u, wave = uint32_t(__builtin_amdgcn_readfirstlane(int(threadIdx.x >> 6)));
    uint32_t (&s_vis)[kQueueBlock] = s_vis_all[wave];
    float (&s_ray)[5][kQueueBlock] = s_ray_all[wave];
    uint8_t (&s_list)[kQueueBlock] = s_list_all[wave];
    float4 (&s_cut)[kCutMax][2] = s_cut_all[wave];
    const unsigned long long t_cost0 = a.co.wave_cost ? __builtin_readcyclecounter() : 0ull;
    if constexpr (!STATS) {
        if (a.co.order_out && blockIdx.x == 0u) order_blocks_by_cost<WAVES>(a.co.cost_prev, a.co.order_blocks, a.co.order_out, reinterpret_cast<uint32_t *>(s_dyn));
    }
    int *stack = s_dyn + wave * (stack_levels + 3u) * kQueueBlock + lane;
    stack[0] = kStackSentinel;
    const uint32_t W = a.width, H = a.height;
    uint32_t x, y;
    const uint32_t block_tile = a.co.block_order ? a.co.block_order[blockIdx.x] : blockIdx.x;
    tile_pixel<WAVES>(block_tile, block_tiles_x, wave, lane, a.row_begin, tile_rows, x, y, a.col_begin);
    const bool in_range = x < a.col_end && y < a.row_end && (lane >> 3) < tile_rows;
    bool covered = false;
    float depth = 0.0f;
    if (in_range) {
        depth = a.depth[size_t(y) * W + x];
        covered = depth != 0.0f;
        if (!covered) store_rg16f(a.shadow_ao, W, x, y, 1.0f, 1.0f);
    }
    s_vis[lane] = 0;
    const uint32_t first_kind = a.tp.shadow_enable ? 0u : 1u;
    const uint32_t last_kind = a.tp.ao_spp;
    const bool ao_only = first_kind != 0u;
    const bool kind_bits = last_kind <= 30u;
    const f3 L = -f3{ a.pfd.directional_light.direction[0], a.pfd.directional_light.direction[1], a.pfd.directional_light.direction[2] };
    f3 omin = f3{ 3.0e38f, 3.0e38f, 3.0e38f }, omax = f3{ -3.0e38f, -3.0e38f, -3.0e38f };
    float ao_reach = 0.0f;
    if (covered) {
        const float u = (float(x) + 0.5f) / float(W);
        const float v = (float(y) + 0.5f) / float(H);
        const f3 P = get_world_space_position(a.pfd, depth, u, v);
        const uint2 nraw = reinterpret_cast<const uint2 *>(a.normals)[size_t(y) * W + x];
        const f3 N = f3{ half_bits_to_float(uint16_t(nraw.x & 0xffffu)), half_bits_to_float(uint16_t(nraw.x >> 16)), half_bits_to_float(uint16_t(nraw.y & 0xffffu)) };
        const f3 origin = P + N * a.tp.normal_bias;
        s_ray[0][lane] = origin.x; s_ray[1][lane] = origin.y; s_ray[2][lane] = origin.z;
        s_ray[3][lane] = __uint_as_float(nraw.x); s_ray[4][lane] = __uint_as_float(nraw.y);
        if (ao_only) ao_reach = a.tp.ao_tmax * onb_norm_bound(N);
        omin = origin; omax = origin;
// ... 66 lines not shown
                const uint32_t nd = uint32_t(__popcll(dmask));
                const uint32_t r = lane_rank(idle);
                const bool thief = ((idle >> lane) & 1ull) && r < nd;
                const uint32_t d = thief ? uint32_t(s_list[r]) : lane;
                const int drow = __shfl(sbase, int(d)) + 1;
                const int link = (stack - lane + d)[(thief ? uint32_t(drow) : 0u) * kQueueBlock];
                const float t_ox = __shfl(ro.x, int(d)), t_oy = __shfl(ro.y, int(d)), t_oz = __shfl(ro.z, int(d));
                const float t_dx = __shfl(rd.x, int(d)), t_dy = __shfl(rd.y, int(d)), t_dz = __shfl(rd.z, int(d));
                const float t_ix = __shfl(rinv.x, int(d)), t_iy = __shfl(rinv.y, int(d)), t_iz = __shfl(rinv.z, int(d));
                const float t_nx = __shfl(noi.x, int(d)), t_ny = __shfl(noi.y, int(d)), t_nz = __shfl(noi.z, int(d));
                const float t_ax = COMPACT ? 0.0f : __shfl(ainv.x, int(d)), t_ay = COMPACT ? 0.0f : __shfl(ainv.y, int(d)), t_az = COMPACT ? 0.0f : __shfl(ainv.z, int(d));
                const float t_tmax = __shfl(tmax, int(d));
                const uint32_t t_pk = uint32_t(__shfl(int(pix | (kind << 8)), int(d)));
                wave_lds_sync();
                if (donor && lane_rank(dmask) < n_idle) {
                    ++sbase;
                    stack[uint32_t(sbase) * kQueueBlock] = kStackSentinel;
                }
                if (thief) {
                    ro = f3{ t_ox, t_oy, t_oz }; rd = f3{ t_dx, t_dy, t_dz }; rinv = f3{ t_ix, t_iy, t_iz }; noi = f3{ t_nx, t_ny, t_nz };
                    if (!COMPACT) ainv = f3{ t_ax, t_ay, t_az };
                    tmax = t_tmax; pix = t_pk & 0xffu; kind = t_pk >> 8;
                    cur = link; sp = 0; sbase = 0; emask = 0;
                    has = true;
                }
                if (stats) ++n_refills;
            }
        }
        if (!__any(has)) break;
#ifdef VHR_K1_COUNT_TRIPS
        if (stats) ++n_drain_trips;
#endif
        __builtin_amdgcn_s_setprio(3);
        const unsigned long long t1 = stats ? __builtin_readcyclecounter() : 0ull;
        bool found = false;
        const uint32_t nodes_before = n_nodes, tris_before = n_tris;
        const uint32_t walkers_in = uint32_t(__popcll(__ballot(has && cur >= 0)));
        while (has && cur >= 0) {
            if (uint32_t(__popcll(__ballot(true))) * 16u <= walkers_in * early_exit) break;
            ++n_nodes;
            float tn0, tn1, tf0, tf1;
            int2 links;
            if (COMPACT) {
                const uint4 *np = reinterpret_cast<const uint4 *>(reinterpret_cast<const char *>(a.scene.nodes16) + uint32_t(cur));
                const uint4 c0 = np[0], c1 = np[1];
                box_pair_ch16(c0.x, c0.y, c0.z, c0.w, c1.x, c1.y, rinv, noi, tmin_v, tmax, tn0, tn1, tf0, tf1);
                links = int2{ int(c1.z), int(c1.w) };
            } else {
                const Node48Words nw = load_node48(a.scene.nodes48, cur);
                links = nw.links;
                box_pair_ch(nw.q0, nw.q1, nw.q2, rinv, ainv, noi, tmin_v, tmax, tn0, tn1, tf0, tf1);
            }
            const unsigned long long h0 = cmp_le_mask(tn0, tf0), h1 = cmp_le_mask(tn1, tf1);
            const unsigned long long enter0 = h0 & (~h1 | cmp_le_mask(tn0, tn1));
            const int nearc = select_mask(links.y, links.x, enter0), farc = select_mask(links.x, links.y, enter0);
            int *const row = stack + min(uint32_t(sp), stack_levels + 1u) * kQueueBlock;
            int top = row[0];
            row[kQueueBlock] = farc;
            if (__any(uint32_t(sp) >= stack_levels)) {
                if (SPILL && uint32_t(sp) > stack_levels) top = spill[(uint32_t(sp) - 1u - stack_levels) & uint32_t(kSpillStack - 1)];
                if (uint32_t(sp) >= stack_levels) {
                    if (SPILL && uint32_t(sp) - stack_levels < uint32_t(kSpillStack)) spill[uint32_t(sp) - stack_levels] = farc;
                    else overflow |= uint32_t((h0 & h1) >> lane) & 1u;
                }
            }
            cur = select_mask(top, nearc, h0 | h1);
            {
                int t;
                unsigned long long carry_out;
                asm("v_addc_co_u32_e64 %0, %1, %2, -1, %3" : "=v"(t), "=s"(carry_out) : "v"(sp), "s"(h0));
                asm("v_addc_co_u32_e64 %0, %1, %2, 0, %3" : "=v"(sp), "=s"(carry_out) : "v"(t), "s"(h1));
            }
        }
#ifdef VHR_K1_COUNT_IDLE
        if (stats) {
            const uint32_t mine = n_nodes - nodes_before;
            uint32_t tot = mine;
            for (int off = 32; off > 0; off >>= 1) tot = max(tot, uint32_t(__shfl_xor(int(tot), off)));
            const bool holder = has && cur < 0 && cur != kStackSentinel;
            uint32_t w = mine, hl = holder ? tot - mine : 0u, fr = holder ? 0u : tot - mine;
            for (int off = 32; off > 0; off >>= 1) { w += uint32_t(__shfl_xor(int(w), off)); hl += uint32_t(__shfl_xor(int(hl), off)); fr += uint32_t(__shfl_xor(int(fr), off)); }
            n_drain_le4 += w; n_drain_le8 += hl; n_drain_le16 += fr;
        }
#endif
        const unsigned long long t2 = stats ? __builtin_readcyclecounter() : 0ull;
        auto test_leaf = [&](const int code) {
            const uint32_t vv = ~uint32_t(code);
            const uint32_t first = vv >> 2, count = (vv & 3u) + 1u;
            ++n_leaves;
            const BvhTri *const leaf = a.scene.tris + first;
            for (uint32_t i = 0; i < count; ++i) {
                ++n_tris;
                const float4 ta = reinterpret_cast<const float4 *>(leaf + i)[0], tb = reinterpret_cast<const float4 *>(leaf + i)[1];
                const float tcx = reinterpret_cast<const float *>(leaf + i)[8];
                const f3 v0 = f3{ ta.x, ta.y, ta.z }, e1 = f3{ ta.w, tb.x, tb.y }, e2 = f3{ tb.z, tb.w, tcx };
                float ct, cu, cv;
                if (mt_candidate(ro, rd, v0, e1, e2, tmin, tmax, ct, cu, cv)) {
                    if (solution_consistent(ro, rd, v0, e1, e2, ct, cu, cv)) {
                        if constexpr (FILTER == kFilterAlpha) { if (gbuf_discarded(a.scene, first + i, cu, cv)) continue; }
                        if constexpr (FILTER == kFilterMask) {
                            if ((uint32_t(a.masks.prim_masks[leaf[i].prim]) & (kind == 0 ? a.masks.shadow : a.masks.ao)) == 0u) continue;
                            if (a.masks.alpha && gbuf_discarded(a.scene, first + i, cu, cv)) continue;
                        }
                        found = true;
                        break;
                    }
                    atomicOr(&s_vis[pix], kRedoPixel);
                }
// ... 318 lines not shown
        }
    }
    if constexpr (STATS) {
        RayStats *const rs = a.stats + 1;
        uint32_t n_nodes = wc.nodes, n_leaves = wc.leaves, n_tris = wc.triangles;
        for (int off = 32; off > 0; off >>= 1) { n_nodes += uint32_t(__shfl_xor(int(n_nodes), off)); n_leaves += uint32_t(__shfl_xor(int(n_leaves), off)); n_tris += uint32_t(__shfl_xor(int(n_tris), off)); }
        if (lane == 0) {
            atomicAdd(&rs->node_visits, (unsigned long long)n_nodes);
            atomicAdd(&rs->leaf_visits, (unsigned long long)n_leaves);
            atomicAdd(&rs->triangle_tests, (unsigned long long)n_tris);
            atomicAdd(&rs->wave_iterations, (unsigned long long)wc.wave_trips);
            atomicAdd(&rs->unique_rays, (unsigned long long)(ncov + second_rays));
            atomicAdd(&rs->covered_pixels, (unsigned long long)ncov);
            atomicAdd(&rs->second_bounce_rays, (unsigned long long)second_rays);
            atomicAdd(&rs->refills, (unsigned long long)wc.refills);
            atomicAdd(&rs->waves, 1ull);
            atomicAdd(&rs->cycles_total, __builtin_readcyclecounter() - t_walk0);
            atomicAdd(&rs->cycles_nodes, t_walk);
        }
    }
    if (a.co.wave_cost && lane == 0) a.co.wave_cost[tile] = uint32_t(min(__builtin_readcyclecounter() - t_cost0, 0xffffffffull));
}

static bool alpha_rays(const vhr_context *ctx) { return ctx->alpha_test_rays != 0 && ctx->scene_can_discard; }


static void issue_raygen(vhr_context *ctx, const RaygenArgs &a_in, const uint32_t width, const uint32_t height, const bool alpha = false, const int filter = kFilterNone) {
    RaygenArgs a = a_in;
    a.co = CostOrderArgs{};
    (void)height;
    ctx->time_begin(kKernelRaygen);
    if (alpha) ++ctx->alpha_launches;
    if (filter == kFilterMask) ++ctx->mask_launches;
    if (ctx->options[kOptRaygenVariant] == 0) {
        with_filter(filter, [&](auto al) { launch(ctx, raygen_kernel<decltype(al)::value>, dim3((width + 15) / 16, (a.row_end - a.row_begin + 15) / 16), dim3(kTraceBlock), 0, a); });
    } else {
        const uint32_t rows_traced = a.row_end - a.row_begin;
        uint32_t tile_rows = uint32_t(std::max(0, std::min(8, ctx->options[kOptRaygenTileRows])));
        if (tile_rows == 0u) {
            const uint64_t tiles8 = uint64_t((a.col_end - a.col_begin + 7) / 8) * ((rows_traced + 7) / 8), slots = uint64_t(ctx->cu_count) * 32u;
            tile_rows = tiles8 * 10u < slots * 7u ? 6u : 8u;
        }
        const uint32_t tiles_x = (a.col_end - a.col_begin + 7) / 8, tiles_y = (rows_traced + tile_rows - 1) / tile_rows;
        const int waves = ctx->options[kOptWavesPerBlock];
        const uint32_t wv = waves >= 4 ? 4u : (waves >= 2 ? 2u : 1u);
        const QueueLaunch q = queue_launch(ctx, kOptLdsStackLevels, kOptEarlyExit, wv);
        const bool compact = ctx->options[kOptCompactNodes] != 0 && ctx->nodes16_valid;
        const uint32_t n_blocks = ((tiles_x + wv - 1u) / wv) * tiles_y;
        {
            const uint32_t key = (tiles_x * 2654435761u) ^ (tiles_y * 40503u) ^ (wv << 28) ^ (tile_rows << 24) ^ (a.row_begin * 97u) ^ (a.col_begin * 193u);
            if (!a.stats && q.levels >= 5u) prepare_cost_order(ctx, ctx->cost_order_raygen, n_blocks, wv, key, a.co, { tiles_x, (tiles_x + wv - 1u) / wv, wv, 8u, tile_rows, a.col_begin, a.row_begin });
        }
        const uint32_t steal = uint32_t(std::max(0, std::min(63, ctx->options[kOptRaygenSteal])));
        auto go = [&](auto kernel) { launch(ctx, kernel, dim3(n_blocks), dim3(kQueueBlock * wv), q.lds_bytes, a, q.levels, q.threshold, (tiles_x + wv - 1u) / wv, q.early_exit, tile_rows, steal); };
        auto by_flags = [&](auto waves_c) {
            constexpr int WV = decltype(waves_c)::value;
            with_bool(q.spill, [&](auto sp) {
                constexpr bool SP = decltype(sp)::value;
                if (a.fuse_temporal && compact && !a.stats && filter == kFilterNone) {
                    go(raygen_queue_kernel<WV, true, SP, false, true>);
                    return;
                }
                with_bool(compact, [&](auto co) {
                    with_bool(a.stats != nullptr, [&](auto st) { with_filter(filter, [&](auto al) {
                        go(raygen_queue_kernel<WV, decltype(co)::value, SP, decltype(st)::value, false, decltype(al)::value>);
                    }); });
                });
            });
        };
        if (wv == 4u) by_flags(std::integral_constant<int, 4>{});
        else if (wv == 2u) by_flags(std::integral_constant<int, 2>{});
        else by_flags(std::integral_constant<int, 1>{});
    }
    ctx->time_end(kKernelRaygen);
}

struct DeferredRaygen { RaygenArgs a; uint32_t width, height; };
int flush_deferred_raygen(vhr_context *ctx, const TemporalArgs *fuse) {
    if (!ctx->deferred_raygen) return VHR_OK;
    DeferredRaygen d;
    std::memcpy(&d, ctx->deferred_raygen_blob.data(), sizeof(d));
    ctx->deferred_raygen = false;
    if (fuse) { d.a.fuse_temporal = 1u; d.a.temporal = *fuse; }
    PassDescription *const running = ctx->cur_pass;
    ctx->cur_pass = ctx->deferred_pass;
    issue_raygen(ctx, d.a, d.width, d.height);
    if (ctx->deferred_pass && ctx->deferred_pass->stamped_in_kernel) {
        ctx->pending_end = &ctx->d_stamps[ctx->deferred_pass->stamp_index].end;
        ctx->deferred_pass->timed = true;
    }
    ctx->cur_pass = running;
    ctx->deferred_pass = nullptr;
    if (hipGetLastError() != hipSuccess) return ctx->fail(VHR_ERROR_DEVICE, "raygen kernel launch failed");
    return VHR_OK;
}
bool deferred_raygen_matches(const vhr_context *ctx, const TemporalArgs &t) {
    if (!ctx->deferred_raygen) return false;
    DeferredRaygen d;
    std::memcpy(&d, ctx->deferred_raygen_blob.data(), sizeof(d));
    return t.raytraced == d.a.shadow_ao && static_cast<const void *>(t.normals) == d.a.normals && t.width == d.a.width && t.height == d.a.height &&
           t.col_begin == 0 && t.row_begin == 0 && t.limit_x == d.a.width && t.row_end >= d.a.height && t.limit_y >= d.a.height &&
           d.a.col_begin == 0 && d.a.row_begin == 0 && d.a.col_end == d.a.width && d.a.row_end == d.a.height;
}

int launch_raygen(vhr_context *ctx, const vhr_per_frame_data &pfd, uint32_t width, uint32_t height, const Image &normals,
                  const Image &depth, Image &shadow_ao, Image *reflections) {
    if (width != normals.width || height != normals.height || width != depth.width || height != depth.height ||
        width != shadow_ao.width || height != shadow_ao.height || (reflections && (reflections->width != width || reflections->height != height)))
        return ctx->fail(VHR_ERROR_INVALID_ARGUMENT, "TraceRays: launch size must equal the extent of the pass images");
    RaygenArgs a;
    a.fuse_temporal = 0u;
    a.temporal = TemporalArgs{};
    a.co = CostOrderArgs{};
    a.scene = ctx->device_scene();
    a.pfd = pfd;
    a.tp = ctx->trace_params;
    a.normals = normals.ptr;
    a.depth = static_cast<const float *>(depth.ptr);
    a.shadow_ao = shadow_ao.ptr;
// ... 111 lines not shown
```

vulkanhybridrenderer_amd/csrc/trace_queue.hpp:

```cpp
#pragma once

#include <algorithm>
#include <type_traits>

#include "trace_device.hpp"

namespace vhr {

typedef float f2v __attribute__((ext_vector_type(2)));

__device__ __forceinline__ float hw_min(float a, float b) { float r; asm("v_min_f32 %0, %1, %2" : "=v"(r) : "v"(a), "v"(b)); return r; }
__device__ __forceinline__ float hw_max(float a, float b) { float r; asm("v_max_f32 %0, %1, %2" : "=v"(r) : "v"(a), "v"(b)); return r; }
__device__ __forceinline__ float hw_min3(float a, float b, float c) { float r; asm("v_min3_f32 %0, %1, %2, %3" : "=v"(r) : "v"(a), "v"(b), "v"(c)); return r; }
__device__ __forceinline__ float hw_max3(float a, float b, float c) { float r; asm("v_max3_f32 %0, %1, %2, %3" : "=v"(r) : "v"(a), "v"(b), "v"(c)); return r; }

__device__ __forceinline__ unsigned long long cmp_le_mask(float a, float b) { unsigned long long m; asm("v_cmp_le_f32_e64 %0, %1, %2" : "=s"(m) : "v"(a), "v"(b)); return m; }
__device__ __forceinline__ unsigned long long cmp_gt_i32_mask_s(int uniform_a, int b) { unsigned long long m; asm("v_cmp_gt_i32_e64 %0, %1, %2" : "=s"(m) : "s"(uniform_a), "v"(b)); return m; }
__device__ __forceinline__ unsigned long long cmp_eq_i32_mask_s(int uniform_a, int b) { unsigned long long m; asm("v_cmp_eq_i32_e64 %0, %1, %2" : "=s"(m) : "s"(uniform_a), "v"(b)); return m; }
__device__ __forceinline__ int select_mask(int if_clear, int if_set, unsigned long long m) { int d; asm("v_cndmask_b32_e64 %0, %1, %2, %3" : "=v"(d) : "v"(if_clear), "v"(if_set), "s"(m)); return d; }

__device__ __forceinline__ bool box_test_pk(f2v bx, f2v by, f2v bz, f3 inv, f3 noi, float tmin, float tlimit, float &tnear) {
    const f2v tx = __builtin_elementwise_fma(bx, f2v{ inv.x, inv.x }, f2v{ noi.x, noi.x });
    const f2v ty = __builtin_elementwise_fma(by, f2v{ inv.y, inv.y }, f2v{ noi.y, noi.y });
    const f2v tz = __builtin_elementwise_fma(bz, f2v{ inv.z, inv.z }, f2v{ noi.z, noi.z });
// ... 335 lines not shown
    for (int off = 32; off > 0; off >>= 1) mx = max(mx, uint32_t(__shfl_xor(int(mx), off)));
    if ((t & 63u) == 0u) lds[t >> 6] = mx;
    __syncthreads();
    for (uint32_t w = 0; w < uint32_t(WAVES); ++w) mx = max(mx, lds[w]);
    __syncthreads();
    const float scale = float(C) / float(max(1u, mx));
    auto cls = [&](uint32_t c) { return (C - 1u) - min(C - 1u, uint32_t(float(c) * scale)); };
    uint32_t mine[C];
#pragma unroll
    for (uint32_t c = 0; c < C; ++c) mine[c] = 0;
    for (uint32_t b = b0; b < b1; ++b) {
        const uint32_t k = cls(cost(b));
#pragma unroll
        for (uint32_t c = 0; c < C; ++c) mine[c] += k == c ? 1u : 0u;
    }
#pragma unroll
    for (uint32_t c = 0; c < C; ++c) lds[c * NT + t] = mine[c];
    __syncthreads();
    for (uint32_t off = 1; off < C * NT; off <<= 1) {
        uint32_t v[C];
#pragma unroll
        for (uint32_t c = 0; c < C; ++c) { const uint32_t i = c * NT + t; v[c] = i >= off ? lds[i - off] : 0u; }
        __syncthreads();
#pragma unroll
        for (uint32_t c = 0; c < C; ++c) lds[c * NT + t] += v[c];
        __syncthreads();
    }
    uint32_t pos[C];
#pragma unroll
    for (uint32_t c = 0; c < C; ++c) pos[c] = lds[c * NT + t] - mine[c];
    for (uint32_t b = b0; b < b1; ++b) {
        const uint32_t k = cls(cost(b));
        uint32_t p = 0;
#pragma unroll
        for (uint32_t c = 0; c < C; ++c) { p = k == c ? pos[c] : p; pos[c] += k == c ? 1u : 0u; }
        order[p + 1u == n_blocks ? 0u : p + 1u] = b;
    }
    __syncthreads();
}

struct CostOrderArgs {
    uint32_t *wave_cost = nullptr;
    const uint32_t *block_order = nullptr;
    const uint32_t *cost_prev = nullptr;
    uint32_t *order_out = nullptr;
    uint32_t order_blocks = 0;
};

constexpr uint32_t kNoHit = 0xffffffffu;

struct WalkCounters { uint32_t nodes = 0, leaves = 0, triangles = 0, wave_trips = 0, refills = 0; };

struct NoFlag { __device__ __forceinline__ void operator()(uint32_t) const {} };
template <bool SPILL, bool ALPHA, bool DEFER, bool STATS = false, bool PER_RAY = false, typename Fetch, typename Commit, typename Flag = NoFlag,
          typename Reject = NoReject>
__device__ __forceinline__ void wave_queue_walk(const DeviceScene &sc, int *stack, const uint32_t stack_levels, const uint32_t lane,
                                                const uint32_t total, const uint32_t refill_threshold, const uint32_t early_exit,
                                                const float tmin, const float tmax, const bool any_hit, uint32_t &overflow,
                                                const float4 (*cut)[2], const uint32_t cut_n, Fetch fetch, Commit commit, WalkCounters *wc = nullptr,
                                                Flag flag = Flag{}, Reject reject = Reject{}) {
    f3 ro = f3{ 0, 0, 0 }, rd = f3{ 0, 0, 1 }, rinv = f3{ 0, 0, 0 }, noi = f3{ 0, 0, 0 }, ainv = f3{ 0, 0, 0 };
    float tbest = 0.0f, best_u = 0.0f, best_v = 0.0f;
    uint32_t best_tri = kNoHit, best_flat = 0;
    int cur = 0, sp = 0;
    uint32_t pix = 0, next = 0;
    uint32_t emask = 0;
    bool has = false;
    volatile int spill[SPILL ? kSpillStack : 1];
    float tmin_v = tmin;
    asm volatile("" : "+v"(tmin_v));
    float ray_tmin = tmin, ray_tmax = tmax;
    for (;;) {
        const unsigned long long idle = __ballot(!has);
        const uint32_t n_idle = uint32_t(__popcll(idle));
        if (next < total && (n_idle >= refill_threshold || n_idle == 64u)) {
            const uint32_t r = next + lane_rank(idle);
            next += n_idle;
            if (STATS && lane == 0) ++wc->refills;
            if (!has && r < total) {
                if constexpr (PER_RAY) { fetch(r, pix, ro, rd, ray_tmin, ray_tmax); tmin_v = ray_tmin; }
                else fetch(r, pix, ro, rd);
                f3 bo, bd;
                box_ray(sc, ro, rd, bo, bd);
                rinv = f3{ cull_reciprocal(bd.x), cull_reciprocal(bd.y), cull_reciprocal(bd.z) };
                noi = f3{ -(bo.x * rinv.x), -(bo.y * rinv.y), -(bo.z * rinv.z) };
                ainv = f3{ fabsf(rinv.x), fabsf(rinv.y), fabsf(rinv.z) };
                tbest = ray_tmax; best_tri = kNoHit; best_flat = 0; best_u = 0.0f; best_v = 0.0f;
                cur = 0; sp = 0;
                if (cut_n) cut_to_stack(cut, cut_n, stack, stack_levels, rinv, noi, tmin_v, ray_tmax, cur, sp, emask);
                has = true;
            }
        }
        if (!__any(has)) break;
        const uint32_t walkers_in = uint32_t(__popcll(__ballot(has && cur >= 0)));
        uint32_t my_nodes = 0, my_tris = 0;
        while (has && cur >= 0) {
            if (uint32_t(__popcll(__ballot(true))) * 16u <= walkers_in * early_exit) break;
            if (STATS) ++my_nodes;
            const Node48Words nw = load_node48(sc.nodes48, cur);
            const int2 links = nw.links;
            float tn0, tn1;
            bool h0, h1;
            box_pair_ch(nw.q0, nw.q1, nw.q2, rinv, ainv, noi, tmin_v, tbest, h0, h1, tn0, tn1);
            const bool both = h0 && h1, none = !(h0 || h1);
            const bool first0 = tn0 <= tn1;
            const int nearc = first0 ? links.x : links.y, farc = first0 ? links.y : links.x;
            int *const row = stack + min(uint32_t(sp), stack_levels + 1u) * kQueueBlock;
            int top = row[0];
            row[kQueueBlock] = farc;
            if (__any(uint32_t(sp) >= stack_levels)) {
                if (SPILL && uint32_t(sp) > stack_levels) top = spill[(uint32_t(sp) - 1u - stack_levels) & uint32_t(kSpillStack - 1)];
                if (uint32_t(sp) >= stack_levels) {
                    if (SPILL && uint32_t(sp) - stack_levels < uint32_t(kSpillStack)) spill[uint32_t(sp) - stack_levels] = farc;
                    else overflow |= both ? 1u : 0u;
                }
            }
            cur = both ? nearc : (none ? top : (h0 ? links.x : links.y));
            sp += (both ? 1 : 0) - (none ? 1 : 0);
        }
        if (has && cur < 0 && cur != kStackSentinel) {
            const uint32_t vv = ~uint32_t(cur);
            const uint32_t first = vv >> 2, count = (vv & 3u) + 1u;
            bool done = false;
            if (STATS) ++wc->leaves;
            for (uint32_t i = 0; i < count; ++i) {
                const float4 *tp = reinterpret_cast<const float4 *>(sc.tris + first + i);
                const float4 ta = tp[0], tb = tp[1], tc = tp[2];
                float t, uu, ww;
                if (STATS) ++my_tris;
                const f3 v0 = f3{ ta.x, ta.y, ta.z }, e1 = f3{ ta.w, tb.x, tb.y }, e2 = f3{ tb.z, tb.w, tc.x };
                if (mt_candidate(ro, rd, v0, e1, e2, ray_tmin, ray_tmax, t, uu, ww)) {
                    if (!solution_consistent(ro, rd, v0, e1, e2, t, uu, ww)) {
                        if (DEFER) { flag(pix); continue; }
                        if (!mt_binary64(ro, rd, v0, e1, e2, ray_tmin, ray_tmax, t, uu, ww)) continue;
                    }
                    if (ALPHA && alpha_ignored(sc, first + i, uu, ww)) continue;
                    if constexpr (reject_at_hit<Reject>::value) { if (reject(pix, first + i, uu, ww)) continue; }
                    else if constexpr (Reject::kActive) { if (reject(pix, first + i)) continue; }
                    const uint32_t flat = __float_as_uint(tc.w);
                    if (best_tri == kNoHit || t < tbest || (t == tbest && flat < best_flat)) {
                        tbest = t; best_tri = first + i; best_flat = flat; best_u = uu; best_v = ww;
                    }
                    if (any_hit) { done = true; break; }
                }
            }
            if (done) {
                cur = kStackSentinel;
                emask = 0;
            } else {
                cur = stack[min(uint32_t(sp), stack_levels + 1u) * kQueueBlock];
                if (SPILL && __any(uint32_t(sp) > stack_levels)) {
                    if (uint32_t(sp) > stack_levels) cur = spill[(uint32_t(sp) - 1u - stack_levels) & uint32_t(kSpillStack - 1)];
                }
                --sp;
            }
        }
        if (has && cur == kStackSentinel && emask) {
            const int e = __ffs(int(emask)) - 1;
// ... 112 lines not shown
```

vulkanhybridrenderer_amd/csrc/vhr_internal.hpp:

```cpp
#pragma once

#include <hip/hip_runtime.h>
#include <hip/hip_ext.h>

#include <cstdint>
#include <map>
#include <string>
#include <unordered_map>
#include <vector>

#include "vhr_amd.h"

namespace vhr {

struct BvhNode {
    float box0[6];
    float box1[6];
    int32_t child0, child1;
    int32_t pad[2];
};
static_assert(sizeof(BvhNode) == 64, "BvhNode");

struct BvhNode16 {
    uint16_t c[6];
// ... 93 lines not shown
    std::vector<BvhTri> prev_tris;
    std::vector<uint32_t> prev_saved;
    uint64_t prev_differing = 0;
};

struct DirtyRanges {
    static constexpr uint32_t kMax = 16;
    uint32_t count = 0;
    uint32_t lo[kMax] = {}, hi[kMax] = {};
    void clear() { count = 0; }
    void add(uint32_t first, uint32_t n) {
        if (!n) return;
        uint64_t l[kMax + 1], h[kMax + 1];
        uint32_t m = 0;
        uint64_t nl = first, nh = uint64_t(first) + n;
        bool placed = false;
        for (uint32_t i = 0; i < count; ++i) {
            if (hi[i] < nl) { l[m] = lo[i]; h[m] = hi[i]; ++m; continue; }
            if (lo[i] > nh) {
                if (!placed) { l[m] = nl; h[m] = nh; ++m; placed = true; }
                l[m] = lo[i]; h[m] = hi[i]; ++m;
                continue;
            }
            nl = nl < lo[i] ? nl : lo[i];
            nh = nh > hi[i] ? nh : hi[i];
        }
        if (!placed) { l[m] = nl; h[m] = nh; ++m; }
        if (m > kMax) {
            uint32_t best = 0;
            for (uint32_t i = 1; i + 1 < m; ++i) if (l[i + 1] - h[i] < l[best + 1] - h[best]) best = i;
            h[best] = h[best + 1];
            for (uint32_t i = best + 1; i + 1 < m; ++i) { l[i] = l[i + 1]; h[i] = h[i + 1]; }
            --m;
        }
        count = m;
        for (uint32_t i = 0; i < m; ++i) { lo[i] = uint32_t(l[i]); hi[i] = uint32_t(h[i]); }
    }
    __host__ __device__ bool holds(uint32_t x) const {
        bool in = false;
        for (uint32_t i = 0; i < count; ++i) in = in || (x >= lo[i] && x < hi[i]);
        return in;
    }
    uint64_t covered() const { uint64_t s = 0; for (uint32_t i = 0; i < count; ++i) s += hi[i] - lo[i]; return s; }
};
struct RefitDirty { DirtyRanges vertices, primitives; };

void check_node_forms(const HostBvh &bvh, uint64_t out[4], int threads = 0);
bool nodes16_in_range(const HostBvh &bvh);
uint64_t bvh_fingerprint(const HostBvh &bvh);
uint64_t bvh_forms_fingerprint(const HostBvh &bvh);
void derive_node_forms(HostBvh &bvh, int threads = 0, const std::vector<uint8_t> *only = nullptr);
uint64_t bvh_tree_fingerprint(const HostBvh &bvh);
void build_bvh(const vhr_vertex *vertices, const uint32_t *indices, const vhr_primitive *primitives,
               uint32_t primitive_count, HostBvh &out, int leaf_tris = kMaxLeafTris, int threads = 0, int presplit_percent = 0, int frame_mode = 0);
int device_build_bvh(vhr_context *ctx, const std::vector<uint32_t> &tri_prefix, uint32_t total_tris, int leaf_tris, int presplit_percent, int frame_mode);

enum RefitStat { kRefitCount = 0, kRefitRecords = 1, kRefitNodes = 2, kRefitRecordsOutside = 3, kRefitChildrenOutside = 4, kRefitNonFinite = 5, kRefitHalfNodes = 6, kRefitStatWords = 8 };
bool refit_bvh(const vhr_vertex *vertices, const uint32_t *indices, const vhr_primitive *primitives, uint32_t primitive_count, HostBvh &bvh, uint64_t counts[3], int threads = 0,
               uint32_t motion_epoch = 0);
double bvh_sah_cost(const HostBvh &bvh);
struct RefitPlan;
void free_refit_plan(vhr_context *ctx);
int device_refit_bvh(vhr_context *ctx);
enum PartialStat { kPartialCount = 0, kPartialRecords = 1, kPartialNodes = 2, kPartialForms = 3, kPartialRanAs = 4, kPartialCentreMoved = 5, kPartialVertexRanges = 6,
                   kPartialPrimitiveRanges = 7, kPartialStatWords = 8 };
enum PartialRanAs { kRanDirty = 0, kRanWholeFirst = 1, kRanWholeThreshold = 2 };
constexpr double kPartialRefitMaxShare = 0.3;
bool refit_bvh_partial(const vhr_vertex *vertices, const uint32_t *indices, const vhr_primitive *primitives, uint32_t primitive_count, HostBvh &bvh,
                       const RefitDirty &dirty, uint64_t counts[3], uint64_t out[4], int threads = 0, uint32_t motion_epoch = 0);
int device_refit_bvh_partial(vhr_context *ctx, bool *ran_whole);
bool device_refit_boxes_valid(const vhr_context *ctx);
int device_bvh_sah_cost(vhr_context *ctx, double *cost);
int device_motion_settle(vhr_context *ctx);

enum class PassKind { Graphics, Raytracing, Compute };

struct Stamps { unsigned long long *begin, *prev_end; };
struct PassStampPair { unsigned long long begin, end; };
constexpr int kMaxStampedPasses = 64;
#if defined(__HIPCC__)
__device__ __forceinline__ void vhr_stamp(const Stamps &st) {
    if ((st.begin || st.prev_end) && (blockIdx.x | blockIdx.y | blockIdx.z | threadIdx.x | threadIdx.y | threadIdx.z) == 0u) {
        const unsigned long long t = wall_clock64();
        if (st.begin) *st.begin = t;
        if (st.prev_end) *st.prev_end = t;
    }
}
#endif

struct PassDescription {
    std::string name;
    PassKind kind;
    std::vector<vhr_transient_resource> dependencies, outputs;
    std::vector<std::string> resource_names;
    std::string pipeline_name, raygen;
    std::vector<std::string> miss, closest_hit, any_hit;
    std::vector<std::string> kernels;
    uint32_t push_constant_size = 0;
    vhr_external_pass_callback external_cb = nullptr;
    vhr_raytracing_pass_callback rt_cb = nullptr;
    vhr_compute_pass_callback compute_cb = nullptr;
    void *user = nullptr;
    vhr_external_pass_callback epilogue_cb = nullptr;
    void *epilogue_user = nullptr;
    hipEvent_t ev_begin = nullptr, ev_end = nullptr;
    bool timed = false;
    bool begin_stamped = false, end_on_last_dispatch = false;
    bool stamped_in_kernel = false;
// ... 26 lines not shown
    enum Kind { Temporal, Atrous, Copy } kind;
    TemporalArgs t;
    AtrousArgs a;
    const char *copy_src; char *copy_dst; size_t copy_bytes;
    size_t copy_pitch, copy_row_bytes; uint32_t copy_rows;
    const void *src_base; void *dst_base;
};

struct RayQueryCounters { uint32_t redo_count, overflows; unsigned long long hits; };
struct RayQueryScratch { hipStream_t stream; RayQueryCounters *counters; uint32_t *list; uint64_t capacity; };

struct RayStats {
    unsigned long long unique_rays, covered_pixels, stack_overflows, node_visits, leaf_visits, triangle_tests, wave_iterations, second_bounce_rays;
    unsigned long long cycles_total, cycles_setup, cycles_refill, cycles_nodes, cycles_leaves, refills, waves, drain_iterations;
    unsigned long long cut_entries;
    unsigned long long drain_le4, drain_le8, drain_le16;
    unsigned long long pending_rays, pending_retraces;
};

#define VHR_OPTION_TABLE(X)                                                                                                             \
                            \
    X(kOptRaygenVariant, "raygen_variant", 1, 0, 1)              \
    X(kOptReflectionVariant, "reflection_variant", 1, 0, 1)            \
    X(kOptRaytracedVariant, "raytraced_variant", 1, 0, 1)        \
    X(kOptAtrousVariant, "atrous_variant", 1, 0, 1)              \
                                                                                                                 \
    X(kOptRefillThreshold, "refill_threshold", 16, 1, 64)               \
    X(kOptLdsStackLevels, "lds_stack_levels", 8, 1, 32)          \
    X(kOptReflectionLdsStackLevels, "reflection_lds_stack_levels", 10, 1, 32)  \
    X(kOptWavesPerBlock, "raygen_waves_per_block", 2, 1, 4)         \
    X(kOptCompactNodes, "compact_nodes", 1, 0, 1)                         \
    X(kOptEarlyExit, "raygen_early_exit", 6, 0, 15)              \
    X(kOptReflectionEarlyExit, "reflection_early_exit", 8, 0, 15)  \
    X(kOptRaygenTileRows, "raygen_tile_rows", 0, 0, 8)           \
    X(kOptRaygenCostOrder, "raygen_cost_order", 1, 0, 2)         \
    X(kOptRaygenSteal, "raygen_steal", 8, 0, 63)                 \
                                                                                                                \
    X(kOptAtrousSmallTiles, "atrous_small_tiles", -1, -1, 1)     \
                                                                                                              \
    X(kOptFuseBlits, "fuse_blits", 1, 0, 1)                                        \
    X(kOptSvgfElideUnread, "svgf_elide_unread", 0, 0, 1)         \
    X(kOptSvgfAsyncUnread, "svgf_async_unread", 1, 0, 2)          \
    X(kOptReflectionAsync, "reflection_async", 1, 0, 2)           \
    X(kOptFuseTemporal, "fuse_temporal", 0, 0, 1)                             \
    X(kOptFramesInFlight, "frames_in_flight", 1, 1, 3)                                                      \
                                                                                   \
    X(kOptTraceOverlap, "trace_overlap", 0, 0, 1)                \
    X(kOptShrinkOverlap, "strip_shrink_overlap", 0, 0, 1)            \
                                                                                                                   \
    X(kOptPassTimestamps, "pass_timestamps", 1, 0, 3)            \
    X(kOptKernelTimingStride, "kernel_timing_stride", 1, 1, 1000000)    \
                          \
    X(kOptRayqueryVariant, "variant_rayquery", 1, 0, 1)          \
    X(kOptForwardRasterVariant, "variant_standin_forward_raster", 1, 0, 1)

enum Option {
#define X(e, n, d, lo, hi) e,
    VHR_OPTION_TABLE(X)
#undef X
    kOptCount
};
struct OptionInfo { const char *name; int def, lo, hi; };
inline constexpr OptionInfo kOptionInfo[kOptCount] = {
#define X(e, n, d, lo, hi) { n, d, lo, hi },
    VHR_OPTION_TABLE(X)
#undef X
};

enum KernelKind { kKernelRaygen = 0, kKernelTemporal = 1, kKernelAtrous = 2, kKernelCopy = 3, kKernelReflection = 4, kKernelSsao = 5, kKernelSsaoBlur = 6, kKernelSsr = 7, kKernelAtrousAsync = 8, kKernelRayQuery = 9,
                  kKernelRayqueryForward = 10, kKernelForwardRaster = 11, kKernelKinds = 12,
                  kKernelRefit = 12 };
struct KernelTimer {
    std::vector<hipEvent_t> events;
    size_t used = 0;
    uint64_t seen = 0;
    double total_ms = 0.0;
    uint64_t launches = 0;
};

}

struct vhr_raytracing_execution_context {
    vhr_context *ctx;
    vhr::PassDescription *pass;
    uint32_t resource_idx;
};
struct vhr_compute_execution_context {
    vhr_context *ctx;
    vhr::PassDescription *pass;
    uint32_t resource_idx;
};

struct vhr_context {
    int device = 0;
    bool host_only = false;
    uint32_t width = 0, height = 0;
    hipStream_t stream = nullptr;
    bool own_stream = false;
    std::string error;

    static constexpr uint32_t kMaxGlobalResources = 2048;
    std::vector<vhr::Image> storage_images;
    struct Texture { void *texels; uint32_t w, h; int32_t format; vhr_sampler_info sampler; };
    std::vector<Texture> textures;
    vhr::DeviceTexture *d_textures = nullptr;
    bool textures_dirty = false;
    vhr_per_frame_data per_frame[3] = {};
    uint32_t last_resource_idx = 0;
    vhr_trace_params trace_params = {};

    vhr_vertex *d_vertices = nullptr;
    uint32_t *d_indices = nullptr;
    vhr_primitive *d_primitives = nullptr;
    float *d_normal_matrices = nullptr;
    vhr::BvhNode *d_nodes = nullptr;
    vhr::BvhNode16 *d_nodes16 = nullptr;
    vhr::BvhNodeCH *d_nodes_ch = nullptr;
    vhr::BvhNode48 *d_nodes48 = nullptr;
    uint64_t bvh_fingerprint = 0;
    uint64_t bvh_tree_fingerprint = 0;
    bool bvh_fingerprint_valid = false;
    int alpha_test_rays = 0;
    bool scene_can_discard = false;
    uint32_t alpha_launches = 0;
    std::vector<uint8_t> h_prim_masks;
    uint8_t *d_prim_masks = nullptr;
    uint64_t mask_present[4] = { 0, 0, 0, 1ull << 63 };
    uint64_t masks_not_ff = 0;
    int shadow_ray_mask = 255, ao_ray_mask = 255, reflection_ray_mask = 255;
    uint32_t mask_launches = 0;
    uint32_t rq_mask_ran = 0;
    bool ray_mask_acts(uint32_t m) const {
        for (uint32_t v = 0; v < 256u; ++v)
            if (((mask_present[v >> 6] >> (v & 63u)) & 1u) && (v & m) == 0u) return true;
        return false;
    }
    int object_motion_vectors = 0;
    vhr::BvhTri *d_prev_tris = nullptr;
    uint32_t *d_prev_saved = nullptr;
    uint32_t motion_epoch = 1;
    uint64_t motion_differing = 0;
    uint64_t motion_refit_differing = 0;
    uint64_t motion_launches = 0;
    bool motion_valid() const { return object_motion_vectors && (host_only ? !h_bvh.prev_tris.empty() : d_prev_tris != nullptr); }
    int bvh_host_checks = 0;
    uint64_t bvh_form_checks[4] = { 0, 0, 0, 0 };
    float bvh_centre[3] = { 0, 0, 0 };
    bool nodes16_valid = false;
    vhr::BvhTri *d_tris = nullptr;
    uint32_t vertex_count = 0, index_count = 0, primitive_count = 0, node_count = 0, tri_count = 0, bvh_depth = 0;
    int bvh_leaf_tris = vhr::kDefaultLeafTris;
    int bvh_build_threads = 0;
    int bvh_frame_mode = 1;
    float bvh_frame[9] = { 1, 0, 0, 0, 1, 0, 0, 0, 1 };
    bool bvh_frame_on = false;
    int bvh_presplit = 0;
    int bvh_presplit_level = -1;
    int bvh_builder = 1;
    int bvh_builder_used = 0;
    int bvh_device_max_depth = vhr::kMaxBvhDepth;
    double bvh_build_ms = 0.0, geometry_upload_ms = 0.0;
    double bvh_check_ms = 0.0;
    bool refit_pending = false;
    uint64_t refit_stats[vhr::kRefitStatWords] = {};
    double refit_times_ms[4] = { 0, 0, 0, 0 };
    double sah_cost_built = 0.0;
    bool sah_cost_built_valid = false;
    vhr::RefitPlan *refit_plan = nullptr;
    vhr::RefitDirty refit_dirty;
    uint64_t partial_stats[vhr::kPartialStatWords] = {};
    std::vector<uint32_t> prim_tri_prefix;
    std::vector<vhr_vertex> h_vertices;
    std::vector<uint32_t> h_indices;
    std::vector<vhr_primitive> h_primitives;
    vhr::HostBvh h_bvh;
    int refuse_if_stale(const char *who) {
        if (!refit_pending) return VHR_OK;
        return fail(VHR_ERROR_GRAPH, std::string(who) + ": geometry updates are pending (vhr_update_vertices / vhr_update_primitive_transforms): call vhr_refit_geometry first");
    }

    std::map<std::string, vhr::PassDescription> pass_descriptions;
    std::vector<std::string> registration_order;
    std::vector<std::string> execution_order;
    std::unordered_map<std::string, vhr::Image> images;
    std::unordered_map<std::string, std::string> compute_kernel_owner;
    bool built = false;

    uint32_t row_begin = 0, row_end = 0, overlap = 0, halo = 0;
    uint32_t col_begin = 0, col_end = 0, halo_cols = 0;

    int frames_in_flight = 1;
    hipStream_t front_stream = nullptr;
    hipEvent_t front_done[3] = { nullptr, nullptr, nullptr }, back_done[3] = { nullptr, nullptr, nullptr };
    bool back_pending[3] = { false, false, false };
    size_t front_passes = 0;
    uint32_t cur_slot = 0;
    int sync_streams();
    hipStream_t side_stream = nullptr;
    hipEvent_t side_ready = nullptr, side_done = nullptr;
#ifndef VHR_JOIN_EVENT_FLAGS
#define VHR_JOIN_EVENT_FLAGS (hipEventDisableTiming | hipEventDisableSystemFence)
#endif
    bool side_pending = false;
    const void *side_reads[2] = { nullptr, nullptr }, *side_writes = nullptr;
    bool async_atrous = false;
    int join_side();
    hipStream_t refl_stream = nullptr;
    hipEvent_t refl_ready = nullptr, refl_done = nullptr;
// ... 112 lines not shown
```

vulkanhybridrenderer_amd/lib.py:

```python
import ctypes as C
import os

import numpy as np

from . import abi

_HERE = os.path.dirname(os.path.abspath(__file__))
LIB_PATH = os.path.join(_HERE, "libvhr_amd.so")

EXPORTS = [
    "vhr_create", "vhr_destroy", "vhr_resize", "vhr_last_error", "vhr_synchronize", "vhr_version", "vhr_abi_struct_sizes",
    "vhr_default_trace_params", "vhr_update_geometry", "vhr_upload_texture_from_data", "vhr_upload_new_storage_image",
    "vhr_destroy_storage_image", "vhr_update_per_frame_ubo", "vhr_set_trace_params", "vhr_graph_destroy_resources",
    "vhr_graph_add_graphics_pass", "vhr_graph_add_raytracing_pass", "vhr_graph_add_compute_pass", "vhr_graph_build",
    "vhr_graph_execute", "vhr_graph_gather_performance_statistics", "vhr_graph_get_pass_time_ms",
    "vhr_graph_get_execution_order", "vhr_graph_contains_image", "vhr_graph_get_image_format",
    "vhr_graph_set_pass_epilogue", "vhr_graph_bind_external_image", "vhr_trace_rays", "vhr_compute_get_display_size",
    "vhr_compute_dispatch", "vhr_compute_blit_image_storage_to_transient", "vhr_compute_blit_image_transient_to_storage",
    "vhr_compute_blit_image_storage_to_storage", "vhr_hybrid_create", "vhr_hybrid_destroy", "vhr_hybrid_build",
    "vhr_hybrid_rebuild", "vhr_hybrid_get_push_constants", "vhr_hybrid_last_error", "vhr_hybrid_state_size", "vhr_hybrid_save_state",
    "vhr_hybrid_load_state", "vhr_get_last_per_frame_ubo", "vhr_get_display_size",
    "vhr_get_transient_image", "vhr_get_storage_image", "vhr_upload_transient_image", "vhr_download_transient_image",
    "vhr_upload_storage_image", "vhr_download_storage_image", "vhr_standin_gbuffer", "vhr_standin_gbuffer_with_albedo", "vhr_standin_composition", "vhr_standin_shadow_map", "vhr_set_strip", "vhr_set_tile",
    "vhr_standin_raytraced_composition", "vhr_raytraced_create", "vhr_raytraced_destroy", "vhr_raytraced_build", "vhr_raytraced_rebuild",
    "vhr_raytraced_last_error", "vhr_standin_rayquery_forward", "vhr_rayquery_create", "vhr_rayquery_destroy", "vhr_rayquery_build",
    "vhr_rayquery_rebuild", "vhr_rayquery_last_error", "vhr_standin_forward_raster", "vhr_forward_raster_create", "vhr_forward_raster_destroy",
    "vhr_forward_raster_build", "vhr_forward_raster_rebuild", "vhr_forward_raster_last_error", "vhr_get_transient_image_samples",
    "vhr_set_ray_statistics", "vhr_get_ray_statistics", "vhr_get_bvh_statistics", "vhr_get_current_stream", "vhr_get_bvh_builder", "vhr_get_bvh_presplit_level", "vhr_get_bvh_frame", "vhr_get_bvh_form_checks", "vhr_get_bvh_fingerprint", "vhr_get_bvh_tree_fingerprint", "vhr_get_bvh_forms_fingerprint", "vhr_set_kernel_timing",
    "vhr_get_kernel_time", "vhr_set_option", "vhr_get_option", "vhr_option_count", "vhr_option_info", "vhr_get_traversal_statistics", "vhr_source_fingerprint", "vhr_debug_wave_lifetimes", "vhr_get_reflection_statistics", "vhr_get_binary64_statistics", "vhr_debug_ray_triangle", "vhr_get_traversal_cycles", "vhr_get_drain_statistics", "vhr_get_build_times", "vhr_atrous_overlap", "vhr_atrous_output_extent", "vhr_strip_plan_make",
    "vhr_strip_plan_exchanges", "vhr_tile_grid_choose", "vhr_tile_plan_make", "vhr_tile_plan_make_weighted", "vhr_get_tile_cost_map", "vhr_tile_plan_exchanges", "vhr_tile_plan_replan", "vhr_comm_replan", "vhr_comm_get_unique_id", "vhr_comm_use_library", "vhr_comm_library", "vhr_comm_create", "vhr_comm_create_tiled", "vhr_comm_destroy", "vhr_comm_last_error", "vhr_comm_exchange_raytraced",
    "vhr_comm_start_frame_exchanges", "vhr_comm_finish_frame_exchanges",
    "vhr_calibration_stream_read", "vhr_ray_query", "vhr_get_ray_query_statistics", "vhr_ray_query_struct_layout",
    "vhr_update_vertices", "vhr_update_primitive_transforms", "vhr_refit_geometry", "vhr_get_refit_statistics", "vhr_get_refit_times",
    "vhr_get_bvh_sah_cost", "vhr_refit_geometry_partial", "vhr_get_partial_refit_statistics",
    "vhr_get_object_motion_statistics", "vhr_debug_triangle_records",
    "vhr_set_primitive_masks", "vhr_get_primitive_masks", "vhr_ray_query_masked", "vhr_get_ray_mask_statistics",
]

PATH_PREFIXES = ("hybrid", "raytraced", "rayquery", "forward_raster")


class VhrError(RuntimeError):
    pass


class CreateInfo(C.Structure):
    _fields_ = [("device", C.c_int32), ("width", C.c_uint32), ("height", C.c_uint32), ("stream", C.c_void_p),
                ("flags", C.c_uint32)]


class TransientImage(C.Structure):
    _fields_ = [("type", C.c_int32), ("width", C.c_uint32), ("height", C.c_uint32), ("format", C.c_int32),
                ("binding", C.c_uint32), ("clear_value", C.c_float * 4), ("multisampled", C.c_int32)]


class TransientResource(C.Structure):
    _fields_ = [("type", C.c_int32), ("name", C.c_char_p), ("image", TransientImage)]


class HitShader(C.Structure):
    _fields_ = [("closest_hit", C.c_char_p), ("any_hit", C.c_char_p)]


class RaytracingPipelineDescription(C.Structure):
    _fields_ = [("name", C.c_char_p), ("raygen_shader", C.c_char_p), ("miss_shaders", C.POINTER(C.c_char_p)),
                ("miss_shader_count", C.c_uint32), ("hit_shaders", C.POINTER(HitShader)), ("hit_shader_count", C.c_uint32)]


class ComputePipelineDescription(C.Structure):
    _fields_ = [("kernels", C.POINTER(C.c_char_p)), ("kernel_count", C.c_uint32), ("push_constant_size", C.c_uint32)]


class ImageInfo(C.Structure):
    _fields_ = [("device_ptr", C.c_void_p), ("width", C.c_uint32), ("height", C.c_uint32), ("format", C.c_int32),
                ("bytes_per_pixel", C.c_uint32)]


class CompositionDesc(C.Structure):
    _fields_ = [("shadow_mode", C.c_int32), ("ambient_occlusion_mode", C.c_int32), ("reflection_mode", C.c_int32),
                ("albedo_image", C.c_char_p), ("normals_image", C.c_char_p), ("motion_image", C.c_char_p), ("depth_image", C.c_char_p),
                ("shadow_ao_image", C.c_char_p), ("reflections_image", C.c_char_p), ("output_storage_image", C.c_int32),
                ("ssao_image", C.c_char_p), ("shadow_map_image", C.c_char_p)]


class RayqueryForwardDesc(C.Structure):
    _fields_ = [("output_storage_image", C.c_int32), ("depth_image", C.c_char_p), ("primary_hits", C.c_void_p), ("positions", C.c_void_p),
                ("shadowed", C.c_void_p)]

# ... 158 lines not shown
    L.vhr_get_traversal_cycles.argtypes = [vp, C.POINTER(u64)]
    L.vhr_get_reflection_statistics.argtypes = [vp, C.POINTER(u64)]
    L.vhr_get_binary64_statistics.argtypes = [vp, C.POINTER(u64)]
    L.vhr_debug_ray_triangle.argtypes = [vp, C.c_void_p, u32, C.c_void_p, C.c_void_p]
    L.vhr_debug_wave_lifetimes.argtypes = [vp, C.POINTER(u32), u32, C.POINTER(u32)]
    L.vhr_source_fingerprint.restype = C.c_char_p
    L.vhr_source_fingerprint.argtypes = []
    L.vhr_get_drain_statistics.argtypes = [vp, C.POINTER(u64)]
    L.vhr_get_option.argtypes = [vp, C.c_char_p, C.POINTER(i32)]
    L.vhr_option_count.restype = i32
    L.vhr_option_count.argtypes = []
    L.vhr_option_info.argtypes = [i32, C.POINTER(C.c_char_p), C.POINTER(i32), C.POINTER(i32), C.POINTER(i32)]
    L.vhr_get_build_times.argtypes = [vp, C.POINTER(C.c_double)]
    L.vhr_atrous_overlap.restype = u32
    L.vhr_atrous_overlap.argtypes = [u32]
    L.vhr_atrous_output_extent.restype = u32
    L.vhr_atrous_output_extent.argtypes = [u32, u32]
    L.vhr_strip_plan_make.argtypes = [u32, u32, u32, u32, u32, C.POINTER(StripPlanC)]
    L.vhr_strip_plan_exchanges.argtypes = [C.POINTER(StripPlanC), u32, C.POINTER(RowExchangeC)]
    L.vhr_tile_grid_choose.argtypes = [u32, u32, u32, u32, C.POINTER(u32), C.POINTER(u32)]
    L.vhr_tile_plan_make.argtypes = [u32, u32, u32, u32, u32, u32, u32, u32, u32, C.POINTER(TilePlanC)]
    L.vhr_tile_plan_make_weighted.argtypes = [u32, u32, u32, u32, u32, u32, u32, u32, u32, vp, u32, u32, u32, C.POINTER(TilePlanC)]
    L.vhr_tile_plan_exchanges.argtypes = [C.POINTER(TilePlanC), u32, u32, C.POINTER(RectExchangeC), u32]
    L.vhr_tile_plan_replan.argtypes = [C.POINTER(TilePlanC), C.POINTER(TilePlanC), C.POINTER(RectExchangeC), u32]
    L.vhr_comm_create_tiled.argtypes = [vp, C.POINTER(TilePlanC), C.c_char_p, C.POINTER(vp)]
    L.vhr_comm_get_unique_id.argtypes = [C.c_char_p]
    L.vhr_comm_create.argtypes = [vp, C.POINTER(StripPlanC), C.c_char_p, C.POINTER(vp)]
    L.vhr_comm_destroy.argtypes = [vp]
    L.vhr_comm_destroy.restype = None
    L.vhr_comm_last_error.argtypes = [vp]
    L.vhr_comm_last_error.restype = C.c_char_p
    L.vhr_comm_exchange_raytraced.argtypes = [vp, C.c_char_p]
    L.vhr_comm_start_frame_exchanges.argtypes = [vp, i32, i32, C.c_char_p, i32, vp]
    L.vhr_comm_finish_frame_exchanges.argtypes = [vp]
    L.vhr_comm_replan.argtypes = [vp, C.POINTER(TilePlanC), i32, i32, i32]
    L.vhr_calibration_stream_read.argtypes = [vp, i32, u32]
    L.vhr_ray_query.argtypes = [vp, vp, u32, u32, vp]
    L.vhr_ray_query_masked.argtypes = [vp, vp, u32, u32, u32, vp, vp]
    L.vhr_set_primitive_masks.argtypes = [vp, u32, u32, vp]
    L.vhr_get_primitive_masks.argtypes = [vp, u32, u32, vp]
    L.vhr_get_ray_mask_statistics.argtypes = [vp, C.POINTER(u64)]
    L.vhr_get_ray_query_statistics.argtypes = [vp, C.POINTER(u64)]
    L.vhr_ray_query_struct_layout.argtypes = [C.POINTER(u32)]
    L.vhr_update_vertices.argtypes = [vp, u32, u32, vp, u32]
    L.vhr_update_primitive_transforms.argtypes = [vp, u32, u32, vp]
    L.vhr_refit_geometry.argtypes = [vp]
    L.vhr_get_refit_statistics.argtypes = [vp, C.POINTER(u64)]
    L.vhr_get_refit_times.argtypes = [vp, C.POINTER(C.c_double)]
    L.vhr_get_bvh_sah_cost.argtypes = [vp, C.POINTER(C.c_double)]
    L.vhr_refit_geometry_partial.argtypes = [vp, u32]
    L.vhr_get_partial_refit_statistics.argtypes = [vp, C.POINTER(u64)]
    L.vhr_get_object_motion_statistics.argtypes = [vp, C.POINTER(u64)]
    L.vhr_debug_triangle_records.argtypes = [vp, i32, C.c_void_p, u32, C.POINTER(u32)]
    L.vhr_set_kernel_timing.argtypes = [vp, i32]
    L.vhr_get_kernel_time.argtypes = [vp, i32, C.POINTER(C.c_double), C.POINTER(u64), i32]
    _lib = L
    return L


NORMALS = "World Space Normals and Object IDs"
MOTION = "Motion Vectors and Metallic Roughness"
DEPTH = "Depth"
RAYTRACED = "Raytraced Shadows and Ambient Occlusion"
REFLECTIONS = "Raytraced Reflections"
DENOISED = "Denoised Raytraced Shadows and Ambient Occlusion"
ALBEDO = "Albedo"
SVGF_SHADER = "hybrid_render_path/svgf.comp"
ATROUS_SHADER = "hybrid_render_path/svgf_atrous_filter.comp"
RAYTRACED_OUTPUT = "RaytracedOutput"
SHADOW_MAP = "Shadow Map"
SSAO_RAW = "Screen Space Ambient Occlusion Raw"
SSAO = "Screen Space Ambient Occlusion"
SSR = "Screen Space Reflections"
SSAO_SHADER = "hybrid_render_path/ssao.comp"
SSAO_BLUR_SHADER = "hybrid_render_path/ssao_blur.comp"
SSR_SHADER = "hybrid_render_path/ssr.comp"

ATTACHMENT_IMAGE, SAMPLED_IMAGE, STORAGE_IMAGE = 0, 1, 2
UPDATE_DEVICE_MEMORY = 2
REFIT_FORCE_PARTIAL = 1


def transient(name, fmt, binding, kind=STORAGE_IMAGE, width=0, height=0, clear=(0, 0, 0, 0)):
    r = TransientResource()
    r.type = 0
    r.name = name.encode()
    r.image.type = kind
    r.image.width, r.image.height = width, height
    r.image.format = fmt
    r.image.binding = binding
    r.image.clear_value = (C.c_float * 4)(*clear)
    return r


def render_output(binding=0):
    return transient("RENDER_OUTPUT", 0, binding, ATTACHMENT_IMAGE)


_NP_FORMATS = {abi.FORMAT_R16G16B16A16_SFLOAT: (np.uint16, 4), abi.FORMAT_R16G16_SFLOAT: (np.uint16, 2),
               abi.FORMAT_D32_SFLOAT: (np.float32, 1), abi.FORMAT_B8G8R8A8_UNORM: (np.uint8, 4),
               abi.FORMAT_R8G8B8A8_UNORM: (np.uint8, 4), abi.FORMAT_R8G8B8A8_SRGB: (np.uint8, 4),
               abi.FORMAT_B8G8R8A8_SRGB: (np.uint8, 4)}


def _p(a):
    return a.ctypes.data_as(C.c_void_p)
# ... 52 lines not shown
    def update_vertices(self, vertices, first_vertex=0):
        v = np.ascontiguousarray(vertices)
        assert v.dtype == abi.vertex_dtype
        self.check(self.L.vhr_update_vertices(self.handle, int(first_vertex), len(v), _p(v) if len(v) else None, 0), "update_vertices")

    def update_vertices_device(self, vertices_ptr, count, first_vertex=0):
        self.check(self.L.vhr_update_vertices(self.handle, int(first_vertex), int(count), vertices_ptr or None, UPDATE_DEVICE_MEMORY), "update_vertices_device")

    def update_primitive_transforms(self, transforms, first_primitive=0):
        t = np.ascontiguousarray(transforms, np.float32).reshape(-1, 16)
        self.check(self.L.vhr_update_primitive_transforms(self.handle, int(first_primitive), len(t), _p(t) if len(t) else None), "update_primitive_transforms")

    def set_primitive_masks(self, masks, first_primitive=0):
        m = np.ascontiguousarray(masks, np.uint8).reshape(-1)
        self.check(self.L.vhr_set_primitive_masks(self.handle, int(first_primitive), len(m), _p(m) if len(m) else None), "set_primitive_masks")

    def primitive_masks(self, first_primitive=0, count=None):
        n = getattr(self, "_primitive_count", 0) - int(first_primitive) if count is None else int(count)
        out = np.zeros(max(n, 0), np.uint8)
        self.check(self.L.vhr_get_primitive_masks(self.handle, int(first_primitive), len(out), _p(out) if len(out) else None), "primitive_masks")
        return out

    def ray_mask_statistics(self):
        out = (C.c_uint64 * 4)()
        self.check(self.L.vhr_get_ray_mask_statistics(self.handle, out), "ray_mask_statistics")
        return [int(x) for x in out]

    def refit_geometry(self):
        self.check(self.L.vhr_refit_geometry(self.handle), "refit_geometry")

    def refit_geometry_partial(self, force=False):
        self.check(self.L.vhr_refit_geometry_partial(self.handle, REFIT_FORCE_PARTIAL if force else 0), "refit_geometry_partial")

    def partial_refit_statistics(self):
        out = (C.c_uint64 * 8)()
        self.check(self.L.vhr_get_partial_refit_statistics(self.handle, out), "partial_refit_statistics")
        return dict(partial_refits=int(out[0]), dirty_records=int(out[1]), dirty_nodes=int(out[2]), forms_rewritten=int(out[3]), ran_as=int(out[4]),
                    centre_moved=int(out[5]), vertex_ranges=int(out[6]), primitive_ranges=int(out[7]))

    def object_motion_statistics(self):
        out = (C.c_uint64 * 4)()
        self.check(self.L.vhr_get_object_motion_statistics(self.handle, out), "object_motion_statistics")
        return dict(active=int(out[0]), differing_records=int(out[1]), motion_launches=int(out[2]))

    def triangle_records(self, previous=False):
        import numpy as np
        n = C.c_uint32(0)
        rc = self.L.vhr_debug_triangle_records(self.handle, 1 if previous else 0, None, 0, C.byref(n))
        if rc != -1 or n.value == 0:
            self.check(rc, "triangle_records")
        out = np.zeros((n.value, 9), np.float32)
        self.check(self.L.vhr_debug_triangle_records(self.handle, 1 if previous else 0, out.ctypes.data, n.value, C.byref(n)), "triangle_records")
        return out

    def refit_statistics(self):
        out = (C.c_uint64 * 8)()
        self.check(self.L.vhr_get_refit_statistics(self.handle, out), "refit_statistics")
        return dict(refits=int(out[0]), records=int(out[1]), nodes=int(out[2]), records_outside=int(out[3]), children_outside=int(out[4]),
                    non_finite=int(out[5]), half_nodes=int(out[6]), upward_launches=int(out[7]))

    def refit_times_ms(self):
        out = (C.c_double * 4)()
        self.check(self.L.vhr_get_refit_times(self.handle, out), "refit_times")
        return tuple(float(v) for v in out)

    def bvh_sah_cost(self):
        out = (C.c_double * 2)()
        self.check(self.L.vhr_get_bvh_sah_cost(self.handle, out), "bvh_sah_cost")
        return float(out[0]), float(out[1])

    def upload_scene(self, scene):
        for t in scene.textures:
            self.upload_texture_from_data(t["rgba8"], t["format"], (t["mag"], t["min"], t["address_u"], t["address_v"]))
        self.update_geometry(scene.vertices, scene.indices, scene.primitives)

    def upload_texture_from_data(self, rgba8, fmt=abi.FORMAT_R8G8B8A8_UNORM, sampler=None):
        img = np.ascontiguousarray(rgba8, np.uint8)
        s = (C.c_int32 * 4)(*sampler) if sampler is not None else None
        return self.check(self.L.vhr_upload_texture_from_data(self.handle, img.shape[1], img.shape[0], _p(img), fmt, s),
                          "UploadTextureFromData")

    def upload_new_storage_image(self, width, height, fmt):
        r = self.L.vhr_upload_new_storage_image(self.handle, width, height, fmt)
        if r < -1:
            self.check(r, "UploadNewStorageImage")
        return r

    def destroy_storage_image(self, idx):
        self.check(self.L.vhr_destroy_storage_image(self.handle, idx), "DestroyStorageImage")

    def update_per_frame_ubo(self, resource_idx, pfd):
        a = np.ascontiguousarray(pfd)
        assert a.dtype == abi.per_frame_dtype
        self.check(self.L.vhr_update_per_frame_ubo(self.handle, resource_idx, _p(a)), "UpdatePerFrameUBO")

    def set_trace_params(self, tp):
        a = np.ascontiguousarray(tp)
        assert a.dtype == abi.trace_params_dtype
        self.check(self.L.vhr_set_trace_params(self.handle, _p(a)), "set_trace_params")

    def set_strip(self, row_begin, row_end, overlap=0, halo=None):
        halo = overlap if halo is None else halo
        self.check(self.L.vhr_set_strip(self.handle, row_begin, row_end, overlap, halo), "set_strip")

    def set_tile(self, col_begin, col_end, row_begin, row_end, overlap=0, halo_rows=None, halo_cols=None):
        halo_rows = overlap if halo_rows is None else halo_rows
# ... 617 lines not shown
```

Baseline: 13440.

## Order BVH children by surface-area term and use fixed child order for any-hit rays

The host and device BVH builders can now swap each inner node's children so the child with the larger surface-area term sits in slot 0, with ties broken by first triangle index. This is on by default. A new any_hit_order option, also on by default, makes the shadow/AO raygen kernel and any-hit ray queries always visit child 0 first instead of sorting children by entry distance. The aim is to reach occluders sooner on any-hit rays and to drop the per-node distance comparison. Closest-hit traversal efficiency could suffer if such rays end up on this fixed order, and more template variants are compiled. A debug API that reads back BVH nodes is also added.

```diff
diff --git a/include/vhr_amd.h b/include/vhr_amd.h
--- a/include/vhr_amd.h
+++ b/include/vhr_amd.h
@@ -261,6 +261,7 @@
 int vhr_debug_wave_lifetimes(vhr_context *ctx, uint32_t *out, uint32_t capacity, uint32_t *count);
 int vhr_debug_ray_triangle(vhr_context *ctx, const float *pairs, uint32_t count, uint32_t *hit, float *tuv);
 int vhr_debug_triangle_records(vhr_context *ctx, int32_t previous, float *out, uint32_t capacity_triangles, uint32_t *count);
+int vhr_debug_bvh_nodes(vhr_context *ctx, void *node_words, uint32_t capacity_nodes, uint32_t *nodes, uint32_t *record_flat, uint32_t capacity_records, uint32_t *records);
 int vhr_get_tile_cost_map(vhr_context *ctx, uint32_t *out, uint32_t cols, uint32_t rows);
 
 int vhr_get_traversal_statistics(vhr_context *ctx, uint64_t out[4]);
diff --git a/vulkanhybridrenderer_amd/csrc/bvh_build.cpp b/vulkanhybridrenderer_amd/csrc/bvh_build.cpp
--- a/vulkanhybridrenderer_amd/csrc/bvh_build.cpp
+++ b/vulkanhybridrenderer_amd/csrc/bvh_build.cpp
@@ -275,7 +275,7 @@
 }
 
 void build_bvh(const vhr_vertex *vertices, const uint32_t *indices, const vhr_primitive *primitives,
-               uint32_t primitive_count, HostBvh &out, int leaf_tris, int threads, int presplit_percent, int frame_mode) {
+               uint32_t primitive_count, HostBvh &out, int leaf_tris, int threads, int presplit_percent, int frame_mode, int child_order) {
     const bool k0trace = std::getenv("VHR_K0_TRACE") != nullptr; auto k0t = std::chrono::steady_clock::now();
     auto lap = [&](const char *what) { if (k0trace) { auto t = std::chrono::steady_clock::now(); std::fprintf(stderr, "K0 %s %.1f ms\n", what, std::chrono::duration<double, std::milli>(t - k0t).count()); k0t = t; } };
     Builder b;
@@ -460,6 +460,10 @@
         derive_node_forms(out, threads);
         return;
     }
+    auto first_in_order = [&](int32_t id) {
+        while (b.nodes[id].left >= 0) id = b.nodes[id].left;
+        return b.nodes[id].first;
+    };
     std::vector<int32_t> bfs_index(b.nodes.size(), -1);
     std::vector<int32_t> bfs_order;
     std::queue<int32_t> q;
@@ -481,6 +485,8 @@
         const TmpNode &l = b.nodes[t.left], &r = b.nodes[t.right];
         set_child(node, 0, l, l.left >= 0 ? bfs_index[t.left] : bvh_math::leaf_link(leaf_pos[t.left], l.count));
         set_child(node, 1, r, r.left >= 0 ? bfs_index[t.right] : bvh_math::leaf_link(leaf_pos[t.right], r.count));
+        if (child_order == 1 && bvh_math::child1_goes_first(node.box0, node.child0, first_in_order(t.left), node.box1, node.child1, first_in_order(t.right)))
+            bvh_math::swap_children(node);
         out.nodes[k] = node;
     }
     });
diff --git a/vulkanhybridrenderer_amd/csrc/bvh_math.hpp b/vulkanhybridrenderer_amd/csrc/bvh_math.hpp
--- a/vulkanhybridrenderer_amd/csrc/bvh_math.hpp
+++ b/vulkanhybridrenderer_amd/csrc/bvh_math.hpp
@@ -286,6 +286,17 @@
     return area > 0.0 ? sum / area : 0.0;
 }
 
+
+VHR_BM bool child1_goes_first(const float box0[6], int32_t link0, uint32_t first0, const float box1[6], int32_t link1, uint32_t first1) {
+    const double t0 = sah_term(box0, link0), t1 = sah_term(box1, link1);
+    return t1 > t0 || (t1 == t0 && first1 < first0);
+}
+VHR_BM void swap_children(BvhNode &nd) {
+#pragma unroll
+    for (int i = 0; i < 6; ++i) { const float b = nd.box0[i]; nd.box0[i] = nd.box1[i]; nd.box1[i] = b; }
+    const int32_t c = nd.child0; nd.child0 = nd.child1; nd.child1 = c;
+}
+
 #undef VHR_BM
 
 }
diff --git a/vulkanhybridrenderer_amd/csrc/context.cpp b/vulkanhybridrenderer_amd/csrc/context.cpp
--- a/vulkanhybridrenderer_amd/csrc/context.cpp
+++ b/vulkanhybridrenderer_amd/csrc/context.cpp
@@ -440,7 +440,7 @@
         uint32_t acc = 0;
         for (uint32_t p = 0; p < primitive_count; ++p) { prefix[p] = acc; acc += primitives[p].index_count / 3; }
         const auto t0 = std::chrono::steady_clock::now();
-        const int rc = device_build_bvh(ctx, prefix, uint32_t(total_triangles), ctx->bvh_leaf_tris, ctx->bvh_presplit, ctx->bvh_frame_mode);
+        const int rc = device_build_bvh(ctx, prefix, uint32_t(total_triangles), ctx->bvh_leaf_tris, ctx->bvh_presplit, ctx->bvh_frame_mode, ctx->bvh_child_order);
         const auto t1 = std::chrono::steady_clock::now();
         if (rc == VHR_OK) {
             device_built = true;
@@ -460,7 +460,7 @@
     }
     const auto t_build0 = std::chrono::steady_clock::now();
     if (!device_built) {
-        build_bvh(vertices, indices, primitives, primitive_count, bvh, ctx->bvh_leaf_tris, ctx->bvh_build_threads, ctx->bvh_presplit, ctx->bvh_frame_mode);
+        build_bvh(vertices, indices, primitives, primitive_count, bvh, ctx->bvh_leaf_tris, ctx->bvh_build_threads, ctx->bvh_presplit, ctx->bvh_frame_mode, ctx->bvh_child_order);
         ctx->bvh_build_ms = std::chrono::duration<double, std::milli>(std::chrono::steady_clock::now() - t_build0).count();
         ctx->bvh_presplit_level = bvh.presplit_level;
         for (int i = 0; i < 9; ++i) ctx->bvh_frame[i] = bvh.frame[i];
@@ -929,6 +929,11 @@
         ctx->bvh_frame_mode = value;
         return VHR_OK;
     }
+    if (!std::strcmp(key, "bvh_child_order")) {
+        if (value < 0 || value > 1) return ctx->fail(VHR_ERROR_INVALID_ARGUMENT, "bvh_child_order must be 0 (an inner node's children as the split left them) or 1 (the child with the larger surface-area term first)");
+        ctx->bvh_child_order = value;
+        return VHR_OK;
+    }
     if (!std::strcmp(key, "bvh_presplit")) {
         if (value < 0 || value > 400) return ctx->fail(VHR_ERROR_INVALID_ARGUMENT, "bvh_presplit must be 0 (off) or the budget of extra triangle references in percent (1..400)");
         ctx->bvh_presplit = value;
@@ -993,6 +998,7 @@
 int vhr_get_option(vhr_context *ctx, const char *key, int32_t *value) {
     if (!ctx || !key || !value) return VHR_ERROR_INVALID_ARGUMENT;
     if (!std::strcmp(key, "alpha_test_rays")) { *value = ctx->alpha_test_rays; return VHR_OK; }
+    if (!std::strcmp(key, "bvh_child_order")) { *value = ctx->bvh_child_order; return VHR_OK; }
     if (!std::strcmp(key, "object_motion_vectors")) { *value = ctx->object_motion_vectors; return VHR_OK; }
     if (!std::strcmp(key, "shadow_ray_mask")) { *value = ctx->shadow_ray_mask; return VHR_OK; }
     if (!std::strcmp(key, "ao_ray_mask")) { *value = ctx->ao_ray_mask; return VHR_OK; }
@@ -1177,6 +1183,31 @@
     return VHR_OK;
 }
 
+int vhr_debug_bvh_nodes(vhr_context *ctx, void *node_words, uint32_t capacity_nodes, uint32_t *nodes, uint32_t *record_flat, uint32_t capacity_records, uint32_t *records) {
+    if (!ctx || !nodes || !records) return ctx ? ctx->fail(VHR_ERROR_INVALID_ARGUMENT, "vhr_debug_bvh_nodes: null count") : VHR_ERROR_INVALID_ARGUMENT;
+    *nodes = *records = 0;
+    if (ctx->host_only ? ctx->h_bvh.nodes.empty() : (ctx->d_nodes == nullptr || ctx->node_count == 0))
+        return ctx->fail(VHR_ERROR_GRAPH, "vhr_debug_bvh_nodes: no geometry yet (vhr_update_geometry first)");
+    *nodes = ctx->node_count;
+    *records = ctx->tri_count;
+    if (capacity_nodes < ctx->node_count || capacity_records < ctx->tri_count || !node_words || !record_flat)
+        return ctx->fail(VHR_ERROR_INVALID_ARGUMENT, "vhr_debug_bvh_nodes: the tree has " + std::to_string(ctx->node_count) + " nodes and " + std::to_string(ctx->tri_count) + " records");
+    std::vector<BvhTri> fetched;
+    const BvhTri *tris = ctx->h_bvh.tris.data();
+    if (ctx->host_only) {
+        std::memcpy(node_words, ctx->h_bvh.nodes.data(), sizeof(BvhNode) * ctx->node_count);
+    } else {
+        HIP_TRY(ctx, hipSetDevice(ctx->device));
+        { const int src_ = ctx->sync_streams(); if (src_ != VHR_OK) return src_; }
+        fetched.resize(ctx->tri_count);
+        HIP_TRY(ctx, hipMemcpy(node_words, ctx->d_nodes, sizeof(BvhNode) * ctx->node_count, hipMemcpyDeviceToHost));
+        HIP_TRY(ctx, hipMemcpy(fetched.data(), ctx->d_tris, sizeof(BvhTri) * ctx->tri_count, hipMemcpyDeviceToHost));
+        tris = fetched.data();
+    }
+    for (uint32_t k = 0; k < ctx->tri_count; ++k) record_flat[k] = tris[k].flat;
+    return VHR_OK;
+}
+
 int vhr_get_object_motion_statistics(vhr_context *ctx, uint64_t out[4]) {
     if (!ctx || !out) return VHR_ERROR_INVALID_ARGUMENT;
     out[0] = ctx->motion_valid() ? 1u : 0u;
diff --git a/vulkanhybridrenderer_amd/csrc/kernels_bvh.hip b/vulkanhybridrenderer_amd/csrc/kernels_bvh.hip
--- a/vulkanhybridrenderer_amd/csrc/kernels_bvh.hip
+++ b/vulkanhybridrenderer_amd/csrc/kernels_bvh.hip
@@ -95,7 +95,7 @@
 }
 __global__ __launch_bounds__(256) void k0_emit_kernel(const int2 *__restrict__ node_children, const Box6 *__restrict__ node_box, const uint32_t *__restrict__ node_size,
                                                       const uint32_t *__restrict__ kept_rank, const uint32_t *__restrict__ position, uint32_t n, uint32_t total_nodes,
-                                                      uint32_t leaf_tris, BvhNode *__restrict__ nodes) {
+                                                      uint32_t leaf_tris, uint32_t child_order, BvhNode *__restrict__ nodes) {
     const uint32_t node = n + blockIdx.x * 256u + threadIdx.x;
     if (node >= total_nodes || node_size[node] <= leaf_tris) return;
     const int2 ch = node_children[node];
@@ -110,6 +110,9 @@
     bvh_math::pad_slot(b1.lo, b1.hi, out.box1);
     out.child0 = link_of(uint32_t(ch.x));
     out.child1 = link_of(uint32_t(ch.y));
+    if (child_order == 1u && bvh_math::child1_goes_first(out.box0, out.child0, first_triangle(node_children, position, n, uint32_t(ch.x)), out.box1, out.child1,
+                                                         first_triangle(node_children, position, n, uint32_t(ch.y))))
+        bvh_math::swap_children(out);
     nodes[kept_rank[node - n]] = out;
 }
 __global__ __launch_bounds__(256) void k0_kept_flags_kernel(const uint32_t *__restrict__ node_size, uint32_t n, uint32_t total_nodes, uint32_t leaf_tris, uint32_t *__restrict__ flags) {
@@ -877,7 +880,7 @@
         if (e_ != hipSuccess) return ctx->fail(VHR_ERROR_DEVICE, std::string("device K0: ") + #expr + ": " + hipGetErrorString(e_)); \
     } while (0)
 
-int device_build_bvh(vhr_context *ctx, const std::vector<uint32_t> &tri_prefix, uint32_t total_tris, int leaf_tris_in, int presplit_percent, int frame_mode) {
+int device_build_bvh(vhr_context *ctx, const std::vector<uint32_t> &tri_prefix, uint32_t total_tris, int leaf_tris_in, int presplit_percent, int frame_mode, int child_order) {
     uint32_t n = total_tris;
     const uint32_t leaf_tris = uint32_t(std::max(1, std::min(kMaxLeafTris, leaf_tris_in)));
     if (n <= leaf_tris || n < 2u) return VHR_ERROR_OUT_OF_SLOTS;
@@ -1099,7 +1102,7 @@
         K0_TRY(hipcub::DeviceRadixSort::SortPairs(d_sort_work, sort_bytes, d_keys[0], d_keys[1], d_vals[0], d_vals[1], int(n_inner_all), 0, 40, s));
         hipLaunchKernelGGL(k0_bfs_rank_kernel, grid(n_inner), block, 0, s, d_vals[1], n_inner, d_kept_rank);
     }
-    hipLaunchKernelGGL(k0_emit_kernel, grid(n_inner_all), block, 0, s, d_children, d_node_box, d_size, d_kept_rank, d_position, n, total_nodes, leaf_tris, ctx->d_nodes);
+    hipLaunchKernelGGL(k0_emit_kernel, grid(n_inner_all), block, 0, s, d_children, d_node_box, d_size, d_kept_rank, d_position, n, total_nodes, leaf_tris, uint32_t(child_order), ctx->d_nodes);
     hipLaunchKernelGGL(k0_node_bounds_kernel, grid(n_inner), block, 0, s, ctx->d_nodes, n_inner, d_bounds + 6);
     K0_TRY(hipMemcpyAsync(h_bounds, d_bounds, sizeof(h_bounds), hipMemcpyDeviceToHost, s));
     K0_TRY(hipStreamSynchronize(s));
diff --git a/vulkanhybridrenderer_amd/csrc/kernels_ray_query.hip b/vulkanhybridrenderer_amd/csrc/kernels_ray_query.hip
--- a/vulkanhybridrenderer_amd/csrc/kernels_ray_query.hip
+++ b/vulkanhybridrenderer_amd/csrc/kernels_ray_query.hip
@@ -58,7 +58,7 @@
     r[3] = hit ? prim : kNoHit; r[4] = hit ? tri : kNoHit; r[5] = 0u;
 }
 
-template <bool SPILL, int FILTER = kFilterNone>
+template <bool SPILL, int FILTER = kFilterNone, bool ANY_FIXED = false>
 __global__ __launch_bounds__(kQueueBlock * 2) void ray_query_kernel(const RayQueryArgs a, const uint32_t stack_levels, const uint32_t refill_threshold,
                                                                     const uint32_t early_exit, const Stamps st) {
     vhr_stamp(st);
@@ -67,7 +67,7 @@
     const uint64_t first = (uint64_t(blockIdx.x) * 2u + wave) * kQueryWaveRays;
     if (first >= a.count) return;
     const uint32_t base = uint32_t(first), total = uint32_t(min(uint64_t(kQueryWaveRays), uint64_t(a.count) - first));
-    const bool any_hit = a.any_hit != 0u;
+    const bool any_hit = ANY_FIXED || a.any_hit != 0u;
     if (a.scene.node_count == 0) {
         for (uint32_t r = lane; r < total; r += 64u) ray_query_store(a, base + r, any_hit, false, 0.0f, 0.0f, 0.0f, 0u, 0u);
         return;
@@ -76,7 +76,7 @@
     stack[0] = kStackSentinel;
     uint32_t overflow = 0, hits = 0;
     bool flagged = false;
-    wave_queue_walk<SPILL, false, true, false, true>(
+    wave_queue_walk<SPILL, false, true, false, true, ANY_FIXED>(
         a.scene, stack, stack_levels, lane, total, refill_threshold, early_exit, 0.0f, 0.0f, any_hit, overflow, nullptr, 0u,
         [&](uint32_t r, uint32_t &ray, f3 &ro, f3 &rd, float &tmin, float &tmax) {
             ray = base + r;
@@ -181,9 +181,10 @@
     }
     const int filter = launch_filter(mask_acts, alpha);
     ctx->time_begin(kKernelRayQuery);
-    with_bool(ql.spill, [&](auto sp) { with_filter(filter, [&](auto al) {
-        launch(ctx, ray_query_kernel<decltype(sp)::value, decltype(al)::value>, grid, dim3(kQueueBlock * 2), ql.lds_bytes, a, ql.levels, ql.threshold, ql.early_exit);
-    }); });
+    const bool any_fixed = any_hit && ctx->options[kOptAnyHitOrder] != 0;
+    with_bool(ql.spill, [&](auto sp) { with_filter(filter, [&](auto al) { with_bool(any_fixed, [&](auto fx) {
+        launch(ctx, ray_query_kernel<decltype(sp)::value, decltype(al)::value, decltype(fx)::value>, grid, dim3(kQueueBlock * 2), ql.lds_bytes, a, ql.levels, ql.threshold, ql.early_exit);
+    }); }); });
     if (a.scene.node_count != 0) {
         const uint32_t redo_blocks = std::min<uint32_t>((count + kTraceBlock - 1u) / kTraceBlock, uint32_t(ctx->cu_count) * 4u);
         with_filter(filter, [&](auto al) { launch(ctx, ray_query_redo_kernel<decltype(al)::value>, dim3(redo_blocks), dim3(kTraceBlock), 0, a); });
diff --git a/vulkanhybridrenderer_amd/csrc/kernels_trace.hip b/vulkanhybridrenderer_amd/csrc/kernels_trace.hip
--- a/vulkanhybridrenderer_amd/csrc/kernels_trace.hip
+++ b/vulkanhybridrenderer_amd/csrc/kernels_trace.hip
@@ -126,7 +126,7 @@
     }
 }
 
-template <int WAVES, bool COMPACT, bool SPILL, bool STATS, bool FUSE = false, int FILTER = kFilterNone>
+template <int WAVES, bool COMPACT, bool SPILL, bool STATS, bool FUSE = false, int FILTER = kFilterNone, bool NEAR_FIRST = false>
 __global__ __launch_bounds__(kQueueBlock *WAVES) __attribute__((amdgpu_waves_per_eu(VHR_K1_WAVES_MIN, 8))) void raygen_queue_kernel(const RaygenArgs a, const uint32_t stack_levels, const uint32_t refill_threshold,
                                                                           const uint32_t block_tiles_x, const uint32_t early_exit, const uint32_t tile_rows, const uint32_t steal_threshold, const Stamps st) {
     vhr_stamp(st);
@@ -299,8 +299,13 @@
                 box_pair_ch(nw.q0, nw.q1, nw.q2, rinv, ainv, noi, tmin_v, tmax, tn0, tn1, tf0, tf1);
             }
             const unsigned long long h0 = cmp_le_mask(tn0, tf0), h1 = cmp_le_mask(tn1, tf1);
-            const unsigned long long enter0 = h0 & (~h1 | cmp_le_mask(tn0, tn1));
-            const int nearc = select_mask(links.y, links.x, enter0), farc = select_mask(links.x, links.y, enter0);
+            int nearc, farc;
+            if constexpr (NEAR_FIRST) {
+                const unsigned long long enter0 = h0 & (~h1 | cmp_le_mask(tn0, tn1));
+                nearc = select_mask(links.y, links.x, enter0); farc = select_mask(links.x, links.y, enter0);
+            } else {
+                nearc = select_mask(links.y, links.x, h0); farc = links.y;
+            }
             int *const row = stack + min(uint32_t(sp), stack_levels + 1u) * kQueueBlock;
             int top = row[0];
             row[kQueueBlock] = farc;
@@ -725,19 +730,20 @@
             if (!a.stats && q.levels >= 5u) prepare_cost_order(ctx, ctx->cost_order_raygen, n_blocks, wv, key, a.co, { tiles_x, (tiles_x + wv - 1u) / wv, wv, 8u, tile_rows, a.col_begin, a.row_begin });
         }
         const uint32_t steal = uint32_t(std::max(0, std::min(63, ctx->options[kOptRaygenSteal])));
+        const bool near_first = ctx->options[kOptAnyHitOrder] == 0;
         auto go = [&](auto kernel) { launch(ctx, kernel, dim3(n_blocks), dim3(kQueueBlock * wv), q.lds_bytes, a, q.levels, q.threshold, (tiles_x + wv - 1u) / wv, q.early_exit, tile_rows, steal); };
         auto by_flags = [&](auto waves_c) {
             constexpr int WV = decltype(waves_c)::value;
             with_bool(q.spill, [&](auto sp) {
                 constexpr bool SP = decltype(sp)::value;
                 if (a.fuse_temporal && compact && !a.stats && filter == kFilterNone) {
-                    go(raygen_queue_kernel<WV, true, SP, false, true>);
+                    with_bool(near_first, [&](auto nf) { go(raygen_queue_kernel<WV, true, SP, false, true, kFilterNone, decltype(nf)::value>); });
                     return;
                 }
                 with_bool(compact, [&](auto co) {
-                    with_bool(a.stats != nullptr, [&](auto st) { with_filter(filter, [&](auto al) {
-                        go(raygen_queue_kernel<WV, decltype(co)::value, SP, decltype(st)::value, false, decltype(al)::value>);
-                    }); });
+                    with_bool(a.stats != nullptr, [&](auto st) { with_filter(filter, [&](auto al) { with_bool(near_first, [&](auto nf) {
+                        go(raygen_queue_kernel<WV, decltype(co)::value, SP, decltype(st)::value, false, decltype(al)::value, decltype(nf)::value>);
+                    }); }); });
                 });
             });
         };
diff --git a/vulkanhybridrenderer_amd/csrc/trace_queue.hpp b/vulkanhybridrenderer_amd/csrc/trace_queue.hpp
--- a/vulkanhybridrenderer_amd/csrc/trace_queue.hpp
+++ b/vulkanhybridrenderer_amd/csrc/trace_queue.hpp
@@ -411,7 +411,7 @@
 struct WalkCounters { uint32_t nodes = 0, leaves = 0, triangles = 0, wave_trips = 0, refills = 0; };
 
 struct NoFlag { __device__ __forceinline__ void operator()(uint32_t) const {} };
-template <bool SPILL, bool ALPHA, bool DEFER, bool STATS = false, bool PER_RAY = false, typename Fetch, typename Commit, typename Flag = NoFlag,
+template <bool SPILL, bool ALPHA, bool DEFER, bool STATS = false, bool PER_RAY = false, bool CHILD0_FIRST = false, typename Fetch, typename Commit, typename Flag = NoFlag,
           typename Reject = NoReject>
 __device__ __forceinline__ void wave_queue_walk(const DeviceScene &sc, int *stack, const uint32_t stack_levels, const uint32_t lane,
                                                 const uint32_t total, const uint32_t refill_threshold, const uint32_t early_exit,
@@ -462,7 +462,7 @@
             bool h0, h1;
             box_pair_ch(nw.q0, nw.q1, nw.q2, rinv, ainv, noi, tmin_v, tbest, h0, h1, tn0, tn1);
             const bool both = h0 && h1, none = !(h0 || h1);
-            const bool first0 = tn0 <= tn1;
+            const bool first0 = CHILD0_FIRST || tn0 <= tn1;
             const int nearc = first0 ? links.x : links.y, farc = first0 ? links.y : links.x;
             int *const row = stack + min(uint32_t(sp), stack_levels + 1u) * kQueueBlock;
             int top = row[0];
diff --git a/vulkanhybridrenderer_amd/csrc/vhr_internal.hpp b/vulkanhybridrenderer_amd/csrc/vhr_internal.hpp
--- a/vulkanhybridrenderer_amd/csrc/vhr_internal.hpp
+++ b/vulkanhybridrenderer_amd/csrc/vhr_internal.hpp
@@ -169,8 +169,8 @@
 void derive_node_forms(HostBvh &bvh, int threads = 0, const std::vector<uint8_t> *only = nullptr);
 uint64_t bvh_tree_fingerprint(const HostBvh &bvh);
 void build_bvh(const vhr_vertex *vertices, const uint32_t *indices, const vhr_primitive *primitives,
-               uint32_t primitive_count, HostBvh &out, int leaf_tris = kMaxLeafTris, int threads = 0, int presplit_percent = 0, int frame_mode = 0);
-int device_build_bvh(vhr_context *ctx, const std::vector<uint32_t> &tri_prefix, uint32_t total_tris, int leaf_tris, int presplit_percent, int frame_mode);
+               uint32_t primitive_count, HostBvh &out, int leaf_tris = kMaxLeafTris, int threads = 0, int presplit_percent = 0, int frame_mode = 0, int child_order = 0);
+int device_build_bvh(vhr_context *ctx, const std::vector<uint32_t> &tri_prefix, uint32_t total_tris, int leaf_tris, int presplit_percent, int frame_mode, int child_order);
 
 enum RefitStat { kRefitCount = 0, kRefitRecords = 1, kRefitNodes = 2, kRefitRecordsOutside = 3, kRefitChildrenOutside = 4, kRefitNonFinite = 5, kRefitHalfNodes = 6, kRefitStatWords = 8 };
 bool refit_bvh(const vhr_vertex *vertices, const uint32_t *indices, const vhr_primitive *primitives, uint32_t primitive_count, HostBvh &bvh, uint64_t counts[3], int threads = 0,
@@ -303,7 +303,8 @@
     X(kOptKernelTimingStride, "kernel_timing_stride", 1, 1, 1000000)    \
                           \
     X(kOptRayqueryVariant, "variant_rayquery", 1, 0, 1)          \
-    X(kOptForwardRasterVariant, "variant_standin_forward_raster", 1, 0, 1)
+    X(kOptForwardRasterVariant, "variant_standin_forward_raster", 1, 0, 1)    \
+    X(kOptAnyHitOrder, "any_hit_order", 1, 0, 1)
 
 enum Option {
 #define X(e, n, d, lo, hi) e,
@@ -405,6 +406,7 @@
     int bvh_frame_mode = 1;
     float bvh_frame[9] = { 1, 0, 0, 0, 1, 0, 0, 0, 1 };
     bool bvh_frame_on = false;
+    int bvh_child_order = 1;
     int bvh_presplit = 0;
     int bvh_presplit_level = -1;
     int bvh_builder = 1;
diff --git a/vulkanhybridrenderer_amd/lib.py b/vulkanhybridrenderer_amd/lib.py
--- a/vulkanhybridrenderer_amd/lib.py
+++ b/vulkanhybridrenderer_amd/lib.py
@@ -33,7 +33,7 @@
     "vhr_calibration_stream_read", "vhr_ray_query", "vhr_get_ray_query_statistics", "vhr_ray_query_struct_layout",
     "vhr_update_vertices", "vhr_update_primitive_transforms", "vhr_refit_geometry", "vhr_get_refit_statistics", "vhr_get_refit_times",
     "vhr_get_bvh_sah_cost", "vhr_refit_geometry_partial", "vhr_get_partial_refit_statistics",
-    "vhr_get_object_motion_statistics", "vhr_debug_triangle_records",
+    "vhr_get_object_motion_statistics", "vhr_debug_triangle_records", "vhr_debug_bvh_nodes",
     "vhr_set_primitive_masks", "vhr_get_primitive_masks", "vhr_ray_query_masked", "vhr_get_ray_mask_statistics",
 ]
 
@@ -298,6 +298,7 @@
     L.vhr_get_partial_refit_statistics.argtypes = [vp, C.POINTER(u64)]
     L.vhr_get_object_motion_statistics.argtypes = [vp, C.POINTER(u64)]
     L.vhr_debug_triangle_records.argtypes = [vp, i32, C.c_void_p, u32, C.POINTER(u32)]
+    L.vhr_debug_bvh_nodes.argtypes = [vp, C.c_void_p, u32, C.POINTER(u32), C.c_void_p, u32, C.POINTER(u32)]
     L.vhr_set_kernel_timing.argtypes = [vp, i32]
     L.vhr_get_kernel_time.argtypes = [vp, i32, C.POINTER(C.c_double), C.POINTER(u64), i32]
     _lib = L
@@ -456,6 +457,17 @@
         out = np.zeros((n.value, 9), np.float32)
         self.check(self.L.vhr_debug_triangle_records(self.handle, 1 if previous else 0, out.ctypes.data, n.value, C.byref(n)), "triangle_records")
         return out
+
+    def bvh_nodes(self):
+        import numpy as np
+        n, r = C.c_uint32(0), C.c_uint32(0)
+        rc = self.L.vhr_debug_bvh_nodes(self.handle, None, 0, C.byref(n), None, 0, C.byref(r))
+        if rc != -1 or n.value == 0:
+            self.check(rc, "bvh_nodes")
+        words = np.zeros((n.value, 16), np.uint32)
+        flat = np.zeros(r.value, np.uint32)
+        self.check(self.L.vhr_debug_bvh_nodes(self.handle, words.ctypes.data, n.value, C.byref(n), flat.ctypes.data, r.value, C.byref(r)), "bvh_nodes")
+        return words[:, :12].copy().view(np.float32).reshape(-1, 2, 6), words[:, 12:14].copy().view(np.int32), flat
 
     def refit_statistics(self):
         out = (C.c_uint64 * 8)()
```

Result: no change. 13540, median of 6 (+0.7%).
